# jnetter6/RRTQX_3D

Measured on AMD Instinct MI355X. Metric: collision-checked edges/sec + radius-NN queries/sec at N=200k nodes, 256 obs, higher is better.
Workload: dtype f64; 1 GPU; C4: 3D SimpleEdge N=200k M=256 B=16384; n_nodes=200000, n_obstacles=256, batch_per_gpu=16384, global_batch=16384, obstacle_list=spheres, edge=SimpleEdge, fresh_batch_every_step=True, batch_ring=8

## Files before the change

rrtqx_3d_amd/csrc/kernels_finish.hip:

```cpp
#include "nn_device.hpp"

namespace rrtx {

namespace {

constexpr int kFinThreads = 512;
constexpr int kFinQ = kFinThreads / 32;
constexpr int kBigSort = 2048;
constexpr int kHugeSort = 8192;
constexpr int kFinBins = 2048;
constexpr int kFinCrowd = 128;

struct FinishArgs {
  const int *count;
  int nq, bcap;
  const BktRec *bkt;
  BktRec *tmp;
  const HitRec *ovf;
  long long ovf_cap;
  const Scalars *sc;
  int prescattered;
  int want_nearest_fix;
  int64_t *offsets;
  int64_t *needed;
  int32_t *idx;
  double *dist;
  long long out_cap;
  int32_t *owner;
  int32_t *nearest_idx;
  double *nearest_dist;
  int *qhist;
  int n_qhist;
  unsigned *mailbox;
  const double *q;
  uint8_t *hit_out, *hit_in;
  double r_start;
  NearestIndex ni;
};

template <int KSORT>
struct FinLds {
  long long red[kFinThreads / 64];
  long long off[kFinQ + 1];
  int kfull[kFinQ];
  int todo[kFinQ];
  unsigned todo_mask;
  unsigned empty_mask;
  int gcnt;
  int s_idx[KSORT];
  double s_d2[KSORT];
  unsigned char s_fl[KSORT];
  int bins[kFinBins + 1];
  int mm[2 * (kFinThreads / 64)];
  double r_best[kFinThreads / 64];
  int r_besti[kFinThreads / 64];
  NearestScratch ns;
};

__device__ __forceinline__ BktRec load_rec(const FinishArgs &a, int q, long long b, long long j) {
  if (j < a.bcap) return a.bkt[(size_t)q * (size_t)a.bcap + (size_t)j];
  const unsigned long long *p = reinterpret_cast<const unsigned long long *>(a.tmp + b + j);
  BktRec r;
  const unsigned long long w0 = __hip_atomic_load(p, __ATOMIC_RELAXED, __HIP_MEMORY_SCOPE_AGENT);
  const unsigned long long w1 = __hip_atomic_load(p + 1, __ATOMIC_RELAXED, __HIP_MEMORY_SCOPE_AGENT);
  r.idx = (int)(unsigned)(w0 & 0xffffffffull);
  r.pad = (int)(unsigned)(w0 >> 32);
  r.d2 = __longlong_as_double((long long)w1);
  return r;
}

template <int D, int KSORT>
__global__ __launch_bounds__(kFinThreads, KSORT > kBigSort ? 2 : 8) void nn_finish_kernel(FinishArgs a) {
  __shared__ FinLds<KSORT> sm;
  const int t = threadIdx.x, lane = t & 63;
  const int wave = __builtin_amdgcn_readfirstlane(t >> 6);
  const int hl = t & 31, hw = t >> 5;
  const int q0 = (int)blockIdx.x * kFinQ;
  const int q = q0 + hw;
  const bool qv = q < a.nq;

  for (int k = (int)blockIdx.x * kFinThreads + t; k < a.n_qhist; k += (int)gridDim.x * kFinThreads) a.qhist[k] = 0;
  if (blockIdx.x == 0 && t == 0 && a.mailbox) {
    const unsigned long long tot = a.sc->total;
    a.mailbox[0] = tot > 0xffffffffull ? 0xffffffffu : (unsigned)tot;
  }

  if (hl == 0) sm.todo[hw] = 0;
  if (t == 0) sm.empty_mask = 0u;
  int kfull = 0;
  if (qv) kfull = a.count[q];
  const int kInt = 0x7fffffff;
  BktRec e0, e1;
  e0.idx = kInt; e0.pad = 0; e0.d2 = __builtin_inf();
  e1 = e0;
  if (qv && hl < a.bcap) e0 = a.bkt[(size_t)q * (size_t)a.bcap + (size_t)hl];
  unsigned long long psum = 0;
  if (!a.prescattered) {
    const int4 *c4 = reinterpret_cast<const int4 *>(a.count);
    const int n4 = (int)blockIdx.x * (kFinQ / 4);
#pragma unroll 4
    for (int j = t; j < n4; j += kFinThreads) {
      const int4 v = c4[j];
      psum += (unsigned)v.x + (unsigned)v.y;
      psum += (unsigned)v.z + (unsigned)v.w;
    }
  }
  const bool small = kfull <= 64 && kfull <= a.bcap;
  const int kk = (qv && small) ? kfull : 0;
  if (!(hl < kk)) { e0.idx = kInt; e0.d2 = __builtin_inf(); }
  if (hl + 32 < kk) e1 = a.bkt[(size_t)q * (size_t)a.bcap + (size_t)(hl + 32)];
  __builtin_amdgcn_wave_barrier();

  const int m0 = e0.idx, m1 = e1.idx;
  const double d0 = e0.d2, d1 = e1.d2;
  int r0 = half_rank_below<false>(m0, m0), r1 = 0;
  double nbest = d0;
  int nbest_i = m0;
  if (__ballot(kk > 32) != 0ull) {
    r0 += half_rank_below<true>(m1, m0);
    r1 = half_rank_below<true>(m0, m1) + half_rank_below<false>(m1, m1);
    const bool second = (d1 < d0) | ((d1 == d0) & (m1 < m0));
    nbest = second ? d1 : d0;
    nbest_i = second ? m1 : m0;
  }
  if (a.nearest_idx) {
    const double dm = half_min_no_nan(nbest);
    nbest_i = half_min((nbest == dm) ? nbest_i : kInt);
    nbest = dm;
  }

  if (!a.prescattered) {
    psum = wave_sum_last(psum);
    if (lane == 63) sm.red[wave] = (long long)psum;
  }
  if (qv && hl == 0) {
    sm.kfull[hw] = kfull;
    if (!small) sm.todo[hw] = 1;
  }
  if (!qv && hl == 0) sm.kfull[hw] = 0;
  __syncthreads();
  if (wave == 0) {
    long long p = 0;
    if (a.prescattered) {
      p = a.offsets[q0];
    } else {
      for (int w = 0; w < kFinThreads / 64; ++w) p += sm.red[w];
    }
    const int kf = lane < kFinQ ? sm.kfull[lane] : 0;
    const int td = lane < kFinQ ? sm.todo[lane] : 0;
    static_assert(kFinQ == 16, "the sixteen lengths sit in one DPP row");
    const long long v = (long long)row_incl_scan((unsigned long long)kf);
    if (lane < kFinQ) sm.off[lane] = p + v - kf;
    if (lane == kFinQ - 1) sm.off[kFinQ] = p + v;
    const unsigned long long tmb = __ballot(td != 0);
    if (lane == 0) sm.todo_mask = (unsigned)tmb;
  }
  __syncthreads();
  if (!a.prescattered && t <= kFinQ) {
    const int qq = q0 + t;
    if (qq < a.nq) a.offsets[qq] = sm.off[t];
    if (qq == a.nq) {
      a.offsets[qq] = sm.off[t];
      if (a.needed) *a.needed = sm.off[t];
    }
  }

  {
    const long long b = qv ? sm.off[hw] : 0;
    const bool w0 = hl < kk && b + r0 < a.out_cap, w1 = hl + 32 < kk && b + r1 < a.out_cap;
    const bool near = a.nearest_idx != nullptr;
    if (hl < kk) {
      const double s0 = sqrt_rn(d0);
      if (w0) {
        a.idx[b + r0] = m0;
        a.dist[b + r0] = s0;
        if (a.owner) a.owner[b + r0] = q;
        if (a.hit_out) { a.hit_out[b + r0] = e0.pad & 1; a.hit_in[b + r0] = (e0.pad >> 1) & 1; }
      }
      if (near && m0 == nbest_i && d0 == nbest) { a.nearest_idx[q] = m0; a.nearest_dist[q] = s0; }
    }
    if (hl + 32 < kk) {
      const double s1 = sqrt_rn(d1);
      if (w1) {
        a.idx[b + r1] = m1;
        a.dist[b + r1] = s1;
        if (a.owner) a.owner[b + r1] = q;
        if (a.hit_out) { a.hit_out[b + r1] = e1.pad & 1; a.hit_in[b + r1] = (e1.pad >> 1) & 1; }
      }
      if (near && m1 == nbest_i && d1 == nbest) { a.nearest_idx[q] = m1; a.nearest_dist[q] = s1; }
    }
    if (near && qv && small && hl == 0 && kk == 0) {
      if (a.want_nearest_fix) atomicOr(&sm.empty_mask, 1u << hw);
      else { a.nearest_idx[q] = -1; a.nearest_dist[q] = __builtin_inf(); }
    }
  }
  __syncthreads();

  for (unsigned tm = sm.todo_mask; tm != 0u; tm &= tm - 1u) {
    const int g = __ffs((int)tm) - 1;
    const int qq = q0 + g;
    const long long gb = sm.off[g];
    const int gfull = sm.kfull[g];
    long long ge = gb + gfull;
    if (ge > a.out_cap) ge = a.out_cap;
    const int gk = ge > gb ? (int)(ge - gb) : 0;
    if (!a.prescattered && gfull > a.bcap) {
      if (t == 0) sm.gcnt = 0;
      __syncthreads();
      long long total = (long long)a.sc->total;
      if (total > a.ovf_cap) total = a.ovf_cap;
      for (long long i = t; i < total; i += kFinThreads) {
        const HitRec r = a.ovf[i];
        if ((r.owner & 0x3fffffff) == qq) {
          const long long dst = gb + a.bcap + atomicAdd(&sm.gcnt, 1);
          if (dst < a.out_cap) {
            unsigned long long *p = reinterpret_cast<unsigned long long *>(a.tmp + dst);
            __hip_atomic_store(p, (unsigned long long)(unsigned)r.idx | ((unsigned long long)((unsigned)r.owner >> 30) << 32),
                               __ATOMIC_RELAXED, __HIP_MEMORY_SCOPE_AGENT);
            __hip_atomic_store(p + 1, (unsigned long long)__double_as_longlong(r.d2), __ATOMIC_RELAXED,
                               __HIP_MEMORY_SCOPE_AGENT);
          }
        }
      }
      asm volatile("s_waitcnt vmcnt(0)" ::: "memory");
      __syncthreads();
    }
    double best = __builtin_inf();
    int best_i = 0x7fffffff;
    bool placed = false;
    if (KSORT > kBigSort && gk <= KSORT) {
      constexpr int kEpt = KSORT / kFinThreads;
      int my_idx[kEpt], my_fl[kEpt], my_bin[kEpt], my_in[kEpt];
      double my_d2[kEpt];
      int lo = 0x7fffffff, hi = (int)0x80000000;
#pragma unroll
      for (int e = 0; e < kEpt; ++e) {
        const int i = e * kFinThreads + t;
        my_idx[e] = 0x7fffffff; my_fl[e] = 0; my_d2[e] = __builtin_inf(); my_bin[e] = 0; my_in[e] = 0;
        if (i < gk) {
          const BktRec r = load_rec(a, qq, gb, i);
          my_idx[e] = r.idx; my_d2[e] = r.d2; my_fl[e] = r.pad;
          lo = min(lo, r.idx); hi = max(hi, r.idx);
        }
      }
      for (int k = t; k <= kFinBins; k += kFinThreads) sm.bins[k] = 0;
#pragma unroll
      for (int off = 32; off > 0; off >>= 1) { lo = min(lo, __shfl_xor(lo, off)); hi = max(hi, __shfl_xor(hi, off)); }
      if (lane == 0) { sm.mm[2 * wave] = lo; sm.mm[2 * wave + 1] = hi; }
      __syncthreads();
#pragma unroll
      for (int w = 0; w < kFinThreads / 64; ++w) { lo = min(lo, sm.mm[2 * w]); hi = max(hi, sm.mm[2 * w + 1]); }
      const double scale = (double)kFinBins / ((double)hi - (double)lo + 1.0);
#pragma unroll
      for (int e = 0; e < kEpt; ++e) {
        if (e * kFinThreads + t < gk) {
          int b = (int)(((double)my_idx[e] - (double)lo) * scale);
          b = b < 0 ? 0 : (b > kFinBins - 1 ? kFinBins - 1 : b);
          my_bin[e] = b;
          my_in[e] = atomicAdd(&sm.bins[b], 1);
        }
      }
      __syncthreads();
      {
        static_assert(kFinBins == 4 * kFinThreads, "four bins per thread");
        const int c0 = sm.bins[4 * t], c1 = sm.bins[4 * t + 1], c2 = sm.bins[4 * t + 2], c3 = sm.bins[4 * t + 3];
        int v = c0 + c1 + c2 + c3;
        const int mine = v;
#pragma unroll
        for (int off = 1; off < 64; off <<= 1) {
          const int o = __shfl_up(v, off);
          if (lane >= off) v += o;
        }
        int cmax = max(max(c0, c1), max(c2, c3));
#pragma unroll
        for (int off = 32; off > 0; off >>= 1) cmax = max(cmax, __shfl_xor(cmax, off));
        if (lane == 63) { sm.mm[wave] = v; sm.mm[kFinThreads / 64 + wave] = cmax; }
        __syncthreads();
        int pre = v - mine;
        for (int w = 0; w < wave; ++w) pre += sm.mm[w];
        sm.bins[4 * t] = pre; sm.bins[4 * t + 1] = pre + c0; sm.bins[4 * t + 2] = pre + c0 + c1; sm.bins[4 * t + 3] = pre + c0 + c1 + c2;
        if (t == kFinThreads - 1) sm.bins[kFinBins] = pre + mine;
      }
      int crowd = 0;
#pragma unroll
      for (int w = 0; w < kFinThreads / 64; ++w) crowd = max(crowd, sm.mm[kFinThreads / 64 + w]);
      placed = crowd <= kFinCrowd;
      __syncthreads();
     if (placed) {
      int *t_idx = sm.s_idx;
      int *t_pos = reinterpret_cast<int *>(sm.s_d2);
#pragma unroll
      for (int e = 0; e < kEpt; ++e) {
        if (e * kFinThreads + t < gk) {
          const int p = sm.bins[my_bin[e]] + my_in[e];
          t_idx[p] = my_idx[e];
          t_pos[p] = e * kFinThreads + t;
        }
      }
      __syncthreads();
#pragma unroll
      for (int e = 0; e < kEpt; ++e) {
        const int i = e * kFinThreads + t;
        if (i < gk) {
          const int my = my_idx[e];
          const int s0 = sm.bins[my_bin[e]], s1 = sm.bins[my_bin[e] + 1];
          int rank = s0;
          for (int k = s0; k < s1; ++k) {
            const int v = t_idx[k];
            rank += ((v < my) || (v == my && t_pos[k] < i)) ? 1 : 0;
          }
          const double d2 = my_d2[e];
          a.idx[gb + rank] = my;
          a.dist[gb + rank] = sqrt_rn(d2);
          if (a.owner) a.owner[gb + rank] = qq;
          if ((d2 < best) || (d2 == best && my < best_i)) { best = d2; best_i = my; }
          if (a.hit_out) { a.hit_out[gb + rank] = my_fl[e] & 1; a.hit_in[gb + rank] = (my_fl[e] >> 1) & 1; }
        }
      }
     }
    }
    if (placed) {
    } else if (gk <= KSORT) {
      int n2 = 64;
      while (n2 < gk) n2 <<= 1;
      for (int i = t; i < n2; i += kFinThreads) {
        BktRec r;
        r.idx = 0x7fffffff; r.pad = 0; r.d2 = __builtin_inf();
        if (i < gk) r = load_rec(a, qq, gb, i);
        sm.s_idx[i] = r.idx;
        sm.s_d2[i] = r.d2;
        sm.s_fl[i] = (unsigned char)r.pad;
      }
      __syncthreads();
      for (int size = 2; size <= n2; size <<= 1) {
        for (int stride = size >> 1; stride > 0; stride >>= 1) {
          for (int i = t; i < n2; i += kFinThreads) {
            const int j = i ^ stride;
            if (j > i) {
              const bool up = (i & size) == 0;
              const int aa = sm.s_idx[i], cc = sm.s_idx[j];
              if ((aa > cc) == up) {
                sm.s_idx[i] = cc; sm.s_idx[j] = aa;
                const double da = sm.s_d2[i];
                sm.s_d2[i] = sm.s_d2[j]; sm.s_d2[j] = da;
                const unsigned char fa = sm.s_fl[i];
                sm.s_fl[i] = sm.s_fl[j]; sm.s_fl[j] = fa;
              }
            }
          }
          __syncthreads();
        }
      }
      for (int i0 = 0; i0 < gk; i0 += kFinThreads) {
        const int i = i0 + t;
        const bool act = i < gk;
        int my = 0;
        double d2 = 0.0;
        if (act) {
          my = sm.s_idx[i];
          d2 = sm.s_d2[i];
          a.idx[gb + i] = my;
          a.dist[gb + i] = sqrt_rn(d2);
          if (a.owner) a.owner[gb + i] = qq;
          if ((d2 < best) || (d2 == best && my < best_i)) { best = d2; best_i = my; }
          if (a.hit_out) { const int fl = sm.s_fl[i]; a.hit_out[gb + i] = fl & 1; a.hit_in[gb + i] = (fl >> 1) & 1; }
        }
      }
    } else {
      for (int i0 = 0; i0 < gk; i0 += kFinThreads) {
        const int i = i0 + t;
        const bool act = i < gk;
        int my = 0, rank = 0;
        double d2 = 0.0;
        if (act) {
          const BktRec r = load_rec(a, qq, gb, i);
          my = r.idx; d2 = r.d2;
          for (int j = 0; j < gk; ++j) rank += (load_rec(a, qq, gb, j).idx < my) ? 1 : 0;
          a.idx[gb + rank] = my;
          a.dist[gb + rank] = sqrt_rn(d2);
          if (a.owner) a.owner[gb + rank] = qq;
          if ((d2 < best) || (d2 == best && my < best_i)) { best = d2; best_i = my; }
          if (a.hit_out) { a.hit_out[gb + rank] = r.pad & 1; a.hit_in[gb + rank] = (r.pad >> 1) & 1; }
        }
      }
    }
    if (a.nearest_idx) {
#pragma unroll
      for (int off = 32; off > 0; off >>= 1) {
        const double ob = __shfl_xor(best, off);
        const int oi = __shfl_xor(best_i, off);
        if ((ob < best) || (ob == best && oi < best_i)) { best = ob; best_i = oi; }
      }
      if (lane == 0) { sm.r_best[wave] = best; sm.r_besti[wave] = best_i; }
      __syncthreads();
      if (t == 0) {
        for (int w = 1; w < kFinThreads / 64; ++w)
          if ((sm.r_best[w] < best) || (sm.r_best[w] == best && sm.r_besti[w] < best_i)) {
            best = sm.r_best[w]; best_i = sm.r_besti[w];
          }
        if (gk > 0) { a.nearest_idx[qq] = best_i; a.nearest_dist[qq] = sqrt_rn(best); }
        else if (a.want_nearest_fix) atomicOr(&sm.empty_mask, 1u << g);
        else { a.nearest_idx[qq] = -1; a.nearest_dist[qq] = __builtin_inf(); }
      }
    }
    __syncthreads();
  }

  if (a.nearest_idx && a.want_nearest_fix) {
    for (unsigned em = sm.empty_mask; em != 0u; em &= em - 1u) {
      const int g = __ffs((int)em) - 1;
      const int qq = q0 + g;
      const double ex = a.q[(size_t)qq * D + 0], ey = a.q[(size_t)qq * D + 1], ez = a.q[(size_t)qq * D + 2];
      double ew = 0.0;
      if constexpr (D == 4) ew = a.q[(size_t)qq * D + 3];
      double bs;
      int bi;
      block_nearest<D, kFinThreads>(a.ni, ex, ey, ez, ew, a.r_start, sm.ns, bs, bi);
      if (t == 0) { a.nearest_idx[qq] = bi; a.nearest_dist[qq] = sqrt_rn(bs); }
    }
  }
}

}

int launch_nn_finish(rrtx_ctx *ctx, const FinishLaunch &f) {
  const int D = ctx->dim;
  FinishArgs a;
  a.count = f.count; a.nq = f.nq; a.bcap = f.bcap;
  a.bkt = reinterpret_cast<const BktRec *>(f.bkt);
  a.tmp = reinterpret_cast<BktRec *>(f.tmp);
  a.ovf = reinterpret_cast<const HitRec *>(f.ovf);
  a.ovf_cap = f.ovf_cap;
  a.sc = reinterpret_cast<const Scalars *>(f.scalars);
  a.prescattered = f.prescattered ? 1 : 0;
  a.offsets = f.offsets; a.needed = f.needed;
  a.idx = f.idx; a.dist = f.dist; a.out_cap = f.out_cap;
  a.owner = f.owner; a.nearest_idx = f.nearest_idx; a.nearest_dist = f.nearest_dist;
  a.qhist = f.qhist; a.n_qhist = f.n_qhist;
  a.mailbox = f.mailbox;
  a.q = f.q;
  a.r_start = f.r_start;
  a.want_nearest_fix = (f.nearest_idx && ctx->n_wraps == 0) ? 1 : 0;
  a.ni.sx = ctx->sl_d[0]; a.ni.sy = ctx->sl_d[1]; a.ni.sz = ctx->sl_d[2]; a.ni.sw = ctx->sl_d[D == 4 ? 3 : 2];
  a.ni.sid = ctx->sl_id;
  a.ni.chunk_ext = reinterpret_cast<const ChunkExt *>(ctx->chunk_ext.get());
  a.ni.n_nodes = (int)ctx->n_nodes;
  a.ni.n_chunks = (int)((ctx->n_nodes + kSlabChunk - 1) / kSlabChunk);
  a.hit_out = f.hit_out; a.hit_in = f.hit_in;
  const dim3 grid((unsigned)((f.nq + kFinQ - 1) / kFinQ)), block(kFinThreads);
  const bool huge = f.out_cap / (f.nq > 0 ? f.nq : 1) > 512;
  for_dim(D, [&](auto dc) {
    constexpr int DD = decltype(dc)::value;
    if (huge) hipLaunchKernelGGL((nn_finish_kernel<DD, kHugeSort>), grid, block, 0, ctx->stream, a);
    else hipLaunchKernelGGL((nn_finish_kernel<DD, kBigSort>), grid, block, 0, ctx->stream, a);
  });
  RRTX_HIP(ctx, hipGetLastError());
  return RRTX_OK;
}

}
```

rrtqx_3d_amd/csrc/kernels_nn.hip:

```cpp
#include "collide_device.hpp"
#include "nn_device.hpp"

#include <limits>

namespace rrtx {

namespace {

template <int D>
__global__ __launch_bounds__(kScanThreads) void nn_scan_kernel(
    const double *__restrict__ nx, const double *__restrict__ ny, const double *__restrict__ nz,
    const double *__restrict__ nw, int n_nodes, const typename QRecT<D>::type *__restrict__ copies,
    const int2 *__restrict__ meta, const SlotRec *__restrict__ slots, int n_slots, int tile_q, int n_seg,
    int seg_len, const Scalars *__restrict__ sc, HitSink hs) {
  const int seg = blockIdx.x % n_seg;
  const int tile = blockIdx.x / n_seg;
  const int n_copies = sc->n_copies;
  const int q0 = tile * tile_q;
  if (q0 >= n_copies) return;
  const int q1 = min(q0 + tile_q, n_copies);
  const int lane = threadIdx.x & 63;
  const int wave = threadIdx.x >> 6;
  const int node_begin = seg * seg_len;
  const int node_end = min(n_nodes, node_begin + seg_len);
  const double kNaN = __builtin_nan("");

  for (int base = node_begin + wave * kChunk; base < node_end; base += (kScanThreads / 64) * kChunk) {
    double x[kScanU], y[kScanU], z[kScanU], w[kScanU];
    int id[kScanU];
#pragma unroll
    for (int u = 0; u < kScanU; ++u) {
      id[u] = base + u * 64 + lane;
      bool ok = id[u] < node_end;
      x[u] = ok ? nx[id[u]] : kNaN;
      y[u] = ok ? ny[id[u]] : kNaN;
      z[u] = ok ? nz[id[u]] : kNaN;
      if constexpr (D == 4) w[u] = ok ? nw[id[u]] : kNaN; else w[u] = 0.0;
    }
    for (int q = q0; q < q1; ++q) {
      const typename QRecT<D>::type c = copies[q];
      double s[kScanU];
      bool h[kScanU];
      bool any = false;
#pragma unroll
      for (int u = 0; u < kScanU; ++u) {
        if constexpr (D == 4) s[u] = sq4(c.x, c.y, c.z, c.w, x[u], y[u], z[u], w[u]);
        else s[u] = sq3(c.x, c.y, c.z, x[u], y[u], z[u]);
        h[u] = s[u] < c.thr;
        any = any || h[u];
      }
      if (__builtin_expect(__ballot(any) != 0ull, 0)) {
        const int2 m = meta[q];
#pragma unroll
        for (int u = 0; u < kScanU; ++u) {
          bool hu = h[u];
          if (m.y > 0 && hu)
            hu = !seen_by_earlier_slot<D>(slots, n_slots, m.x, m.y, id[u], x[u], y[u], z[u], w[u]);
          emit_hit(hs, hu, m.x, id[u], s[u]);
        }
      }
    }
  }
  (void)lane;
}

constexpr int kMaxQBuckets = 4096;
template <int D>
__global__ __launch_bounds__(256) void nn_place_kernel(
    const typename QRecT<D>::type *__restrict__ copies, const int2 *__restrict__ meta, const int2 *__restrict__ cb,
    const int *__restrict__ qhist, int n_buckets, const Scalars *__restrict__ sc,
    const unsigned long long *__restrict__ node_absmax, double ox, double oy, double oz, double ow,
    typename QRecT<D>::type *__restrict__ copies_s, int2 *__restrict__ meta_s,
    typename QRecFT<D>::type *__restrict__ copies_f) {
  __shared__ int start[kMaxQBuckets];
  __shared__ int wsum[4];
  {
    const int t = threadIdx.x, lane = t & 63, wave = t >> 6;
    static_assert(kMaxQBuckets == 256 * 16, "sixteen counters per thread");
    const int per = (n_buckets + 255) / 256;
    const int b0 = min(t * per, n_buckets), b1 = min(b0 + per, n_buckets);
    int h[16];
    if (per == 16) {
      const int4 *h4 = reinterpret_cast<const int4 *>(qhist + b0);
#pragma unroll
      for (int k = 0; k < 4; ++k) { const int4 v4 = h4[k]; h[4 * k] = v4.x; h[4 * k + 1] = v4.y; h[4 * k + 2] = v4.z; h[4 * k + 3] = v4.w; }
    } else {
#pragma unroll
      for (int k = 0; k < 16; ++k) h[k] = (b0 + k < b1) ? qhist[b0 + k] : 0;
    }
    int local = 0;
#pragma unroll
    for (int k = 0; k < 16; ++k) local += h[k];
    int v = local;
#pragma unroll
    for (int off = 1; off < 64; off <<= 1) {
      const int o = __shfl_up(v, off);
      if (lane >= off) v += o;
    }
    if (lane == 63) wsum[wave] = v;
    __syncthreads();
    int prefix = v - local;
    for (int w = 0; w < wave; ++w) prefix += wsum[w];
#pragma unroll
    for (int k = 0; k < 16; ++k)
      if (b0 + k < b1) { start[b0 + k] = prefix; prefix += h[k]; }
    __syncthreads();
  }
  int i = blockIdx.x * blockDim.x + threadIdx.x;
  const int n_copies = sc->n_copies;
  if (i >= n_copies) {
    if (i < ((n_copies + kQPI - 1) / kQPI) * kQPI) copies_f[i] = never_pass_qrecf<D>();
    return;
  }
  const int2 b = cb[i];
  const int dst = start[b.x] + b.y;
  if ((unsigned)dst >= (unsigned)n_copies) return;
  const typename QRecT<D>::type c = copies[i];
  unsigned long long am = max(*node_absmax, sc->q_absmax);
  copies_s[dst] = c;
  meta_s[dst] = meta[i];
  copies_f[dst] = make_qrecf<D>(c, __longlong_as_double((long long)am), ox, oy, oz, ow);
}

constexpr int kEvSlack = 2048;

template <int D, bool LM, class Emit>
__device__ __forceinline__ void confirm_entry(bool has, int2 en, int n_nodes, const ConfirmArgs &a, const Emit &emit,
                                              const typename QRecT<D>::type *tile_copies = nullptr, int tile_q0 = 0) {
  const typename QRecT<D>::type *__restrict__ copies = static_cast<const typename QRecT<D>::type *>(a.copies);
  typename QRecT<D>::type ce;
  ce.x = 0.0; ce.y = 0.0; ce.z = 0.0; ce.thr = 0.0;
  if constexpr (D == 4) ce.w = 0.0;
  int2 m = make_int2(0, 0);
  const int p0 = has ? en.y : 0;
  if (has) {
    ce = tile_copies ? tile_copies[en.x - tile_q0] : copies[en.x];
    if (Emit::kNeedsOwner || a.n_slots > 1) m = a.meta[en.x];
  }
  constexpr int kH = kScanFU / 2;
#pragma unroll 1
  for (int hv = 0; hv < 2; ++hv) {
    double ex[kH], ey[kH], ez[kH], ew[kH];
    int nid[kH];
    if constexpr (LM) {
      if (a.pos_id) {
        const int4 vi = *reinterpret_cast<const int4 *>(a.pos_id + p0 + kH * hv);
        nid[0] = vi.x; nid[1] = vi.y; nid[2] = vi.z; nid[3] = vi.w;
      } else {
#pragma unroll
        for (int u = 0; u < kH; ++u) nid[u] = p0 + kH * hv + u;
      }
      const double2 *rx = reinterpret_cast<const double2 *>(a.nx + p0 + kH * hv);
      const double2 *ry = reinterpret_cast<const double2 *>(a.ny + p0 + kH * hv);
      const double2 *rz = reinterpret_cast<const double2 *>(a.nz + p0 + kH * hv);
      const double2 *rw = reinterpret_cast<const double2 *>(a.nw + p0 + kH * hv);
#pragma unroll
      for (int v = 0; v < kH / 2; ++v) {
        const double2 vx = rx[v], vy = ry[v], vz = rz[v];
        ex[2 * v] = vx.x; ex[2 * v + 1] = vx.y;
        ey[2 * v] = vy.x; ey[2 * v + 1] = vy.y;
        ez[2 * v] = vz.x; ez[2 * v + 1] = vz.y;
        if constexpr (D == 4) { const double2 vw = rw[v]; ew[2 * v] = vw.x; ew[2 * v + 1] = vw.y; }
        else { ew[2 * v] = 0.0; ew[2 * v + 1] = 0.0; }
      }
    } else {
#pragma unroll
      for (int u = 0; u < kH; ++u) {
        const int pos = p0 + 64 * (kH * hv + u);
        const int pc = (pos < n_nodes) ? pos : 0;
        ex[u] = a.nx[pc]; ey[u] = a.ny[pc]; ez[u] = a.nz[pc];
        if constexpr (D == 4) ew[u] = a.nw[pc]; else ew[u] = 0.0;
        nid[u] = pos;
      }
    }
    double s[kH];
    unsigned hm = 0u;
#pragma unroll
    for (int u = 0; u < kH; ++u) {
      const int pos = LM ? p0 + kH * hv + u : p0 + 64 * (kH * hv + u);
      if constexpr (D == 4) s[u] = sq4(ce.x, ce.y, ce.z, ce.w, ex[u], ey[u], ez[u], ew[u]);
      else s[u] = sq3(ce.x, ce.y, ce.z, ex[u], ey[u], ez[u]);
      bool hu = has && pos < n_nodes && (s[u] < ce.thr);
      if (m.y > 0 && hu)
        hu = !seen_by_earlier_slot<D>(a.slots, a.n_slots, m.x, m.y, nid[u], ex[u], ey[u], ez[u], ew[u]);
      hm |= (hu ? 1u : 0u) << u;
    }
    if constexpr (Emit::kBatch) {
      static_assert(kH == 4, "batch emitters take four nodes at a time");
      emit.batch(en.x, m.x, hm, nid, s);
    } else {
      while (__ballot(hm != 0u) != 0ull) {
        const bool h = hm != 0u;
        const int uu = h ? (__ffs((int)hm) - 1) : 0;
        hm &= hm - 1u;
        double hs2 = s[0];
        int hid = nid[0];
#pragma unroll
        for (int u = 1; u < kH; ++u) { hs2 = (uu == u) ? s[u] : hs2; hid = (uu == u) ? nid[u] : hid; }
        emit(h, en.x, m.x, hid, hs2);
      }
    }
  }
}

constexpr int kConfirmParts = 4;
template <int D, bool LM>
__global__ __launch_bounds__(256) void nn_confirm_kernel(ConfirmArgs a, const int2 *__restrict__ ev,
                                                         const int *__restrict__ ev_cnt, int n_slices,
                                                         int slice_cap, int n_nodes) {
  const int lane = threadIdx.x & 63;
  const int gw = __builtin_amdgcn_readfirstlane((int)blockIdx.x * (int)(blockDim.x >> 6) + (int)(threadIdx.x >> 6));
  const int w = gw / kConfirmParts, part = gw % kConfirmParts;
  if (w >= n_slices) return;
  const int cnt = ev_cnt[w];
  const int2 *__restrict__ mine = ev + (size_t)w * (size_t)slice_cap;
  for (int e0 = 64 * part; e0 < cnt; e0 += 64 * kConfirmParts) {
    const int e = e0 + lane;
    const bool has = e < cnt;
    int2 en = make_int2(0, 0);
    if (has) en = mine[e];
    confirm_entry<D, LM>(has, en, n_nodes, a, GlobalEmit{a.hs});
  }
}


template <int D>
__device__ __forceinline__ typename QRecFT<D>::type uniform_qrecf(const typename QRecFT<D>::type &f) {
  typename QRecFT<D>::type u = f;
  u.x = __int_as_float(__builtin_amdgcn_readfirstlane(__float_as_int(f.x)));
  u.y = __int_as_float(__builtin_amdgcn_readfirstlane(__float_as_int(f.y)));
  u.z = __int_as_float(__builtin_amdgcn_readfirstlane(__float_as_int(f.z)));
  if constexpr (D == 4) u.w = __int_as_float(__builtin_amdgcn_readfirstlane(__float_as_int(f.w)));
  u.thr = __int_as_float(__builtin_amdgcn_readfirstlane(__float_as_int(f.thr)));
  return u;
}
template <int D, int MODE, bool LQ = false>
__device__ __forceinline__ void scan_chunk_f32(const float *__restrict__ fx, const float *__restrict__ fy,
                                               const float *__restrict__ fz, const float *__restrict__ fw,
                                               const float *__restrict__ fpp, const int base, const int node_end,
                                               const typename QRecFT<D>::type *__restrict__ copies_f, const int q0,
                                               const int q1, int2 *__restrict__ mine, int &wn,
                                               const unsigned p_lane = 0u, const unsigned long long vm = ~0ull,
                                               const typename QRecFT<D>::type *lq = nullptr) {
  const int lane = threadIdx.x & 63;
  const float kInf = __builtin_inff();
  constexpr bool LM = MODE != 0;
  float x[kScanFU], y[kScanFU], z[kScanFU], w[kScanFU], pp[kScanFU];
  const unsigned p0 = (MODE == 2) ? p_lane : (unsigned)(base + 8 * lane);
  if constexpr (LM) {
    const float4 *rx = reinterpret_cast<const float4 *>(fx + p0);
    const float4 *ry = reinterpret_cast<const float4 *>(fy + p0);
    const float4 *rz = reinterpret_cast<const float4 *>(fz + p0);
    const float4 *rw = reinterpret_cast<const float4 *>(fw + p0);
    const float4 *rp = reinterpret_cast<const float4 *>(fpp + p0);
#pragma unroll
    for (int v = 0; v < 2; ++v) {
      const float4 vx = rx[v], vy = ry[v], vz = rz[v], vp = rp[v];
      x[4 * v] = vx.x; x[4 * v + 1] = vx.y; x[4 * v + 2] = vx.z; x[4 * v + 3] = vx.w;
      y[4 * v] = vy.x; y[4 * v + 1] = vy.y; y[4 * v + 2] = vy.z; y[4 * v + 3] = vy.w;
      z[4 * v] = vz.x; z[4 * v + 1] = vz.y; z[4 * v + 2] = vz.z; z[4 * v + 3] = vz.w;
      pp[4 * v] = vp.x; pp[4 * v + 1] = vp.y; pp[4 * v + 2] = vp.z; pp[4 * v + 3] = vp.w;
      if constexpr (D == 4) {
        const float4 vw = rw[v];
        w[4 * v] = vw.x; w[4 * v + 1] = vw.y; w[4 * v + 2] = vw.z; w[4 * v + 3] = vw.w;
      } else {
        w[4 * v] = 0.f; w[4 * v + 1] = 0.f; w[4 * v + 2] = 0.f; w[4 * v + 3] = 0.f;
      }
    }
#pragma unroll
    for (int u = 0; u < kScanFU; ++u)
      if ((int)p0 + u >= node_end) { x[u] = 0.f; y[u] = 0.f; z[u] = 0.f; w[u] = 0.f; pp[u] = kInf; }
  } else {
#pragma unroll
    for (int u = 0; u < kScanFU; ++u) {
      const int id = base + u * 64 + lane;
      const bool ok = id < node_end;
      const unsigned idc = (unsigned)(ok ? id : node_end - 1);
      x[u] = fx[idc];
      y[u] = fy[idc];
      z[u] = fz[idc];
      if constexpr (D == 4) w[u] = fw[idc]; else w[u] = 0.f;
      pp[u] = ok ? fpp[idc] : kInf;
    }
  }
  for (int q = q0; q < q1; q += kQPI) {
    typename QRecFT<D>::type c[kQPI];
#pragma unroll
    for (int k = 0; k < kQPI; ++k) {
      if constexpr (LQ) c[k] = uniform_qrecf<D>(lq[q - q0 + k]);
      else c[k] = copies_f[q + k];
    }
    unsigned long long mk[kQPI];
    unsigned long long anym = 0ull;
#pragma unroll
    for (int k = 0; k < kQPI; ++k) {
      float t[kScanFU];
      screen8<D>(c[k], x, y, z, w, pp, t);
      const float m1 = fminf(fminf(t[0], t[1]), t[2]);
      const float m2 = fminf(fminf(t[3], t[4]), t[5]);
      const float m3 = fminf(fminf(t[6], t[7]), m1);
      const float tmin = fminf(m2, m3);
      mk[k] = __ballot(!(tmin > c[k].thr));
      if constexpr (MODE == 2) mk[k] &= vm;
      anym |= mk[k];
    }
    if (anym != 0ull) {
#pragma unroll
      for (int k = 0; k < kQPI; ++k) {
        if (mk[k] == 0ull || q + k >= q1) continue;
        const unsigned before = __builtin_amdgcn_mbcnt_hi((unsigned)(mk[k] >> 32),
                                                          __builtin_amdgcn_mbcnt_lo((unsigned)mk[k], 0u));
        if ((mk[k] >> lane) & 1ull)
          mine[wn + (int)before] = make_int2(q + k, LM ? (int)p0 : base + lane);
        wn += __popcll(mk[k]);
      }
    }
  }
}

template <int D, bool LM, class Emit>
__device__ __forceinline__ void drain_slice_to(const int2 *__restrict__ mine, int &wn, int n_nodes, const ConfirmArgs &a,
                                               const Emit &emit, const typename QRecT<D>::type *tile_copies, int tile_q0) {
  const int lane = threadIdx.x & 63;
  __builtin_amdgcn_fence(__ATOMIC_SEQ_CST, "workgroup");
  for (int e0 = 0; e0 < wn; e0 += 64) {
    const int e = e0 + lane;
    const bool has = e < wn;
    int2 en = make_int2(0, 0);
    if (has) en = mine[e];
    confirm_entry<D, LM>(has, en, n_nodes, a, emit, tile_copies, tile_q0);
  }
  wn = 0;
}

template <int D, bool LM>
__device__ __forceinline__ void drain_slice(const int2 *__restrict__ mine, int &wn, int n_nodes,
                                            const ConfirmArgs *__restrict__ ca) {
  const int lane = threadIdx.x & 63;
  __builtin_amdgcn_fence(__ATOMIC_SEQ_CST, "workgroup");
  const ConfirmArgs a = *ca;
  for (int e0 = 0; e0 < wn; e0 += 64) {
    const int e = e0 + lane;
    const bool has = e < wn;
    int2 en = make_int2(0, 0);
    if (has) en = mine[e];
    confirm_entry<D, LM>(has, en, n_nodes, a, GlobalEmit{a.hs});
  }
  wn = 0;
}

template <int D>
__global__ __launch_bounds__(kScanThreads, 5) void nn_scan_f32_kernel(
    const float *__restrict__ fx, const float *__restrict__ fy, const float *__restrict__ fz,
    const float *__restrict__ fw, const float *__restrict__ fpp, int n_nodes,
    const typename QRecFT<D>::type *__restrict__ copies_f, int tile_q, int n_seg, int seg_len,
    const Scalars *__restrict__ sc, int2 *__restrict__ ev, int *__restrict__ ev_cnt, int slice_cap,
    const ConfirmArgs *__restrict__ ca) {
  const int n_copies = sc->n_copies;
  const int lane = threadIdx.x & 63;
  const int wave = threadIdx.x >> 6;
  const int slice = __builtin_amdgcn_readfirstlane((int)blockIdx.x * (kScanThreads / 64) + wave);
  int2 *__restrict__ mine = ev + (size_t)slice * (size_t)slice_cap;
  int wn = 0;
  const int n_tiles = (n_copies + tile_q - 1) / tile_q;
  const int n_items = n_tiles * n_seg;
  for (int item = blockIdx.x; item < n_items; item += gridDim.x) {
    const int seg = item % n_seg;
    const int tile = item / n_seg;
    const int q0 = tile * tile_q;
    const int q1 = min(q0 + tile_q, n_copies);
    const int node_begin = seg * seg_len;
    const int node_end = min(n_nodes, node_begin + seg_len);
    for (int base = node_begin + wave * kChunkF; base < node_end; base += (kScanThreads / 64) * kChunkF) {
      if (wn + 64 * tile_q > slice_cap) drain_slice<D, false>(mine, wn, n_nodes, ca);
      scan_chunk_f32<D, 0>(fx, fy, fz, fw, fpp, base, node_end, copies_f, q0, q1, mine, wn);
    }
  }
  if (lane == 0) ev_cnt[slice] = wn;
}

constexpr int kTileB = 16;
constexpr int kTbLcap = 96;
constexpr int kTbList = 1024;
constexpr int kTbSlack = 512;

constexpr int kTbGroups = 1024;
template <int D>
struct TileLds {
  int list[kTbList];
  int n_list;
  int glist[kTbGroups];
  int n_groups, gmode;
  double zlo, zhi;
  int wcnt[kScanThreads / 64];
  double lo, hi, ylo, yhi;
  int lcnt[kTileB];
  typename QRecT<D>::type cp[kTileB];
  typename QRecFT<D>::type cf[kTileB];
  int own[kTileB];
  BktRec hrec[kTileB][kTbLcap];
  int snl[kTileB];
  int sok[kTileB];
  int ssl[kTileB][kSphListCap];
  SphRec ssr[kTileB][kSphListCap];
};

struct TileGrid {
  const SlabParams *sp;
  const int *cell_start;
  int n_sorted_chunks;
  int kz;
  int groups;
};

template <int D>
__device__ __forceinline__ bool tile_edge_needed(const ExtendDev &x, const TileLds<D> &sm, int cl, double d2) {
  const double len = sqrt_rn(d2);
  const bool quick = sm.snl[cl] == 0 && sm.sok[cl] != 0 && len > 0.0 && len <= x.r_bound && len < 1e29;
  return !quick && x.m > 0;
}
template <int D>
__device__ __forceinline__ int tile_edge_eval(const ExtendDev &x, const TileLds<D> &sm, bool need, int cl,
                                              const double4 nd, double d2) {
  if (__ballot(need) == 0ull) return 0;
  const typename QRecT<D>::type c = sm.cp[cl];
  bool ho, hi;
  edge_flags(x, need, c.x, c.y, c.z, nd.x, nd.y, nd.z, sqrt_rn(d2), sm.snl[cl], sm.ssl[cl], ho, hi, sm.ssr[cl]);
  return (ho ? 1 : 0) | (hi ? 2 : 0);
}
template <int D>
__device__ __forceinline__ int tile_edge_flags(const ExtendDev &x, const TileLds<D> &sm, bool h, int cl, int id,
                                               double d2) {
  const bool need = h && tile_edge_needed<D>(x, sm, cl, d2);
  if (__ballot(need) == 0ull) return 0;
  double4 nd = make_double4(0.0, 0.0, 0.0, 0.0);
  if (need) nd = x.naos[id];
  return tile_edge_eval<D>(x, sm, need, cl, nd, d2);
}

template <int D, bool EXT>
struct TileEmit {
  static constexpr bool kNeedsOwner = false;
  static constexpr bool kBatch = true;
  __device__ __forceinline__ void batch(int q, int , unsigned hm, const int *id, const double *d2) const {
    const int cl = hm ? q - q0 : 0;
    int base = 0;
    if (hm) base = atomicAdd(&sm.lcnt[cl], __popc(hm));
    unsigned spill = 0u;
#pragma unroll
    for (int u = 0; u < 4; ++u) {
      const bool b = (hm >> u) & 1u;
      if (__ballot(b) == 0ull) continue;
      const int slot = base + __popc(hm & ((1u << u) - 1u));
      if (b && slot < kTbLcap) {
        BktRec br;
        br.idx = id[u]; br.pad = 0; br.d2 = d2[u];
        sm.hrec[cl][slot] = br;
      }
      spill |= (b && slot >= kTbLcap) ? (1u << u) : 0u;
    }
    if (__ballot(spill != 0u) != 0ull) {
#pragma unroll 1
      for (int u = 0; u < 4; ++u) {
        const bool sp = (spill >> u) & 1u;
        if (__ballot(sp) == 0ull) continue;
        int owner = 0, flags = 0;
        if (sp) owner = meta ? meta[q].x : sm.own[cl];
        if constexpr (EXT) flags = tile_edge_flags<D>(x, sm, sp, cl, id[u], d2[u]);
        emit_hits_grouped(hs, sp, owner, id[u], d2[u], flags);
      }
    }
  }
  TileLds<D> &sm;
  const HitSink &hs;
  const int2 *meta;
  const ExtendDev &x;
  int q0;
  __device__ __forceinline__ void operator()(bool h, int q, int , int id, double d2) const {
    const int cl = h ? q - q0 : 0;
    int slot = 0;
    if (h) slot = atomicAdd(&sm.lcnt[cl], 1);
    const bool in_lds = h && slot < kTbLcap;
    if (in_lds) {
      BktRec br;
      br.idx = id; br.pad = 0; br.d2 = d2;
      sm.hrec[cl][slot] = br;
    }
    const bool spill = h && !in_lds;
    if (__ballot(spill) != 0ull) {
      int owner = 0, flags = 0;
      if (spill) owner = meta ? meta[q].x : sm.own[cl];
      if constexpr (EXT) flags = tile_edge_flags<D>(x, sm, spill, cl, id, d2);
      emit_hits_grouped(hs, spill, owner, id, d2, flags);
    }
  }
};

__device__ __forceinline__ int lane_here() {
  int l = (int)(threadIdx.x & 63);
  asm volatile("" : "+v"(l));
  return l;
}
__device__ __forceinline__ int wshfl_i(int v, int src_lane) { return __builtin_amdgcn_ds_bpermute(src_lane << 2, v); }
template <bool MAX>
__device__ __forceinline__ int wave_scan_incl(int v, const int identity) {
#define RRTX_SCAN_STEP(ctrl, rows)                                                              \
  {                                                                                             \
    const int o = __builtin_amdgcn_update_dpp(identity, v, ctrl, rows, 0xf, false);             \
    v = MAX ? max(v, o) : v + o;                                                                \
  }
  RRTX_SCAN_STEP(0x111, 0xf) RRTX_SCAN_STEP(0x112, 0xf) RRTX_SCAN_STEP(0x114, 0xf) RRTX_SCAN_STEP(0x118, 0xf)
  RRTX_SCAN_STEP(0x142, 0xa) RRTX_SCAN_STEP(0x143, 0xc)
#undef RRTX_SCAN_STEP
  return v;
}
template <int N>
__device__ __forceinline__ double row_up_d(double v) {
  const long long b = __double_as_longlong(v);
  const int lo = __builtin_amdgcn_update_dpp((int)(b & 0xffffffffll), (int)(b & 0xffffffffll), 0x100 + N, 0xf, 0xf, false);
  const int hi = __builtin_amdgcn_update_dpp((int)(b >> 32), (int)(b >> 32), 0x100 + N, 0xf, 0xf, false);
  return __longlong_as_double(((long long)hi << 32) | (long long)(unsigned)lo);
}
__device__ __forceinline__ int wave_prev(int v, const int first) {
  return __builtin_amdgcn_update_dpp(first, v, 0x138, 0xf, 0xf, false);
}
__device__ __forceinline__ double wshfl_d(double v, int src_lane) {
  const long long b = __double_as_longlong(v);
  const int lo = __builtin_amdgcn_ds_bpermute(src_lane << 2, (int)(b & 0xffffffffll));
  const int hi = __builtin_amdgcn_ds_bpermute(src_lane << 2, (int)(b >> 32));
  return __longlong_as_double(((long long)hi << 32) | (long long)(unsigned)lo);
}

#ifdef RRTX_TILE_CLOCKS
__device__ unsigned long long g_tile_clk[4096 * 16];
#define RRTX_TILE_CLK_AT(thread, k) do { if (t == (thread)) g_tile_clk[(blockIdx.x & 4095) * 16 + (k)] = wall_clock64(); } while (0)
#else
#define RRTX_TILE_CLK_AT(thread, k) do { } while (0)
#endif
#define RRTX_TILE_CLK(k) RRTX_TILE_CLK_AT(0, k)

struct TilePlace {
  const int *qhist;
  const void *tab;
  const int2 *spill_key;
  int n_buckets, capb, spill_base, n_tab;
};

__device__ __forceinline__ void load_qhist16(const int *__restrict__ qhist, int per, int b0, int b1, int *h) {
  static_assert(kMaxQBuckets == 256 * 16, "sixteen counters per thread");
  if (per == 16) {
    const int4 *h4 = reinterpret_cast<const int4 *>(qhist + b0);
#pragma unroll
    for (int k = 0; k < 4; ++k) { const int4 v4 = h4[k]; h[4 * k] = v4.x; h[4 * k + 1] = v4.y; h[4 * k + 2] = v4.z; h[4 * k + 3] = v4.w; }
  } else {
#pragma unroll
    for (int k = 0; k < 16; ++k) h[k] = (b0 + k < b1) ? qhist[b0 + k] : 0;
  }
}

template <int D, bool EXT, bool SL, bool ONE>
__global__ __launch_bounds__(kScanThreads, 4) void nn_tile_kernel(
    const float *__restrict__ fx, const float *__restrict__ fy, const float *__restrict__ fz,
    const float *__restrict__ fw, const float *__restrict__ fpp, int n_nodes, int n_chunks,
    const ChunkExt *__restrict__ chunk_ext, const typename QRecT<D>::type *__restrict__ copies_s, const typename QRecFT<D>::type *__restrict__ copies_f,
    const Scalars *__restrict__ sc, int n_parts, int2 *__restrict__ ev, int slice_cap,
    const ConfirmArgs a, const ConfirmArgs *__restrict__ ca, const TileGrid tg, const ExtendDev x,
    int *__restrict__ visits, const int n_copies_known, const TilePlace tp) {
  __shared__ TileLds<D> sm;
  const int t = threadIdx.x, lane = t & 63;
  const int wave = __builtin_amdgcn_readfirstlane(t >> 6);
  const int part = blockIdx.x % n_parts;
  const int n_copies = n_copies_known >= 0 ? n_copies_known : sc->n_copies;
  const int n_tiles = (n_copies + kTileB - 1) / kTileB;
  const int slice = (int)blockIdx.x * (kScanThreads / 64) + wave;
  int2 *__restrict__ mine = ev + (size_t)slice * (size_t)slice_cap;
  const int2 *__restrict__ blk = ev + (size_t)blockIdx.x * (kScanThreads / 64) * (size_t)slice_cap;
  int visited = 0;

  const int n_slots = (int)gridDim.x / n_parts;
  const int slot = (int)blockIdx.x / n_parts;
  const int my = (n_slots % 8 == 0) ? (slot % 8) * (n_slots / 8) + slot / 8 : slot;
  for (int tile = my; tile < n_tiles; tile += n_slots) {
    const int q0 = tile * kTileB;
    const int q1 = min(q0 + kTileB, n_copies);
    int wn = 0;

    RRTX_TILE_CLK(0);
    int slot = -1;
    if constexpr (SL) {
      int tq = t;
      asm volatile("" : "+v"(tq));
      const int per = (tp.n_buckets + 255) / 256;
      {
        const int b0 = min(tq * per, tp.n_buckets), b1 = min(b0 + per, tp.n_buckets);
        int h[16];
        load_qhist16(tp.qhist, per, b0, b1, h);
        int local = 0;
#pragma unroll
        for (int k = 0; k < 16; ++k) local += h[k];
        const int incl = wave_scan_incl<false>(local, 0);
        if (lane == 63) sm.wcnt[wave] = incl;
        sm.list[kTileB + tq] = incl - local;
      }
      __syncthreads();
      RRTX_TILE_CLK(11);
      if (wave == 0) {
        const int pos = q0 + lane;
        int rk = -1, bk = 0;
        if (pos < q1) {
          const int w1 = sm.wcnt[0], w2 = w1 + sm.wcnt[1], w3 = w2 + sm.wcnt[2];
          auto start_of = [&](int T) {
            const int w = T >> 6;
            return sm.list[kTileB + T] + (w == 0 ? 0 : (w == 1 ? w1 : (w == 2 ? w2 : w3)));
          };
          int T = 0;
#pragma unroll
          for (int st = 128; st > 0; st >>= 1)
            if (start_of(T + st) <= pos) T += st;
          int p = start_of(T);
          const int b0 = min(T * per, tp.n_buckets), b1 = min(b0 + per, tp.n_buckets);
          int h[16];
          load_qhist16(tp.qhist, per, b0, b1, h);
#pragma unroll
          for (int k = 0; k < 16; ++k) {
            const bool in = pos >= p && pos < p + h[k];
            bk = in ? b0 + k : bk;
            rk = in ? pos - p : rk;
            p += h[k];
          }
          if (rk >= 0 && rk < tp.capb) slot = bk * tp.capb + rk;
        }
        const unsigned long long need = __ballot(rk >= tp.capb);
        if (need != 0ull) {
          const int n_sp = min(sc->n_spill, n_copies);
          unsigned long long todo = need;
          for (int j0 = 0; j0 < n_sp && todo != 0ull; j0 += 64) {
            const int j = j0 + lane;
            const int2 key = j < n_sp ? tp.spill_key[j] : make_int2(-1, -1);
            unsigned long long rem = todo;
            while (rem != 0ull) {
              const int l = __ffsll((long long)rem) - 1;
              rem &= rem - 1ull;
              const int kb = __builtin_amdgcn_readlane(bk, l), kr = __builtin_amdgcn_readlane(rk, l);
              const unsigned long long m = __ballot(key.x == kb && key.y == kr);
              if (m != 0ull) {
                if (lane == l) slot = tp.spill_base + j0 + __ffsll((long long)m) - 1;
                todo &= ~(1ull << l);
              }
            }
          }
        }
      }
    }

    if (t < kTileB) sm.lcnt[t] = 0;
    if (wave == 0) {
      double lo = __builtin_inf(), hi = -__builtin_inf(), ylo = __builtin_inf(), yhi = -__builtin_inf();
      double zlo = __builtin_inf(), zhi = -__builtin_inf();
      if constexpr (SL) {
        if (lane >= q1 - q0 && lane < kTileB) sm.cf[lane] = never_pass_qrecf<D>();
      }
      if (q0 + lane < q1) {
        typename QRecT<D>::type c;
        if constexpr (SL) {
          if ((unsigned)slot < (unsigned)tp.n_tab) {
            const QSlotRec<D> rec = static_cast<const QSlotRec<D> *>(tp.tab)[slot];
            c = rec.q;
            sm.cf[lane] = rec.f;
            sm.own[lane] = rec.owner;
          } else {
            c.x = 0.0; c.y = 0.0; c.z = 0.0; c.thr = -1.0;
            if constexpr (D == 4) { c.w = 0.0; c.pad0 = 0.0; c.pad1 = 0.0; c.pad2 = 0.0; }
            sm.cf[lane] = never_pass_qrecf<D>();
            sm.own[lane] = -1;
          }
        } else {
          c = copies_s[q0 + lane];
        }
        sm.cp[lane] = c;
        if constexpr (EXT) {
          const double rb = x.r_bound >= 0.0 ? x.r_bound : 0.0;
          const double pmax = fmax(fmax(fabs(c.x), fabs(c.y)), fabs(c.z));
          const double base_b = rb + 1e-12 * (pmax + 1.0);
          const bool usable = (pmax < 1e29) && (c.x == c.x) && (c.y == c.y) && (c.z == c.z) && (base_b < 1e29);
          sm.sok[lane] = (usable && x.r_bound >= 0.0) ? 1 : 0;
        }
        const bool can_hit = (c.thr > 0.0) && (c.x - c.x == 0.0) && (c.y - c.y == 0.0) && (c.z - c.z == 0.0);
        if (can_hit) {
          const double R = sqrt_rn(c.thr) * (1.0 + 1e-15);
          const double xa = c.x - R, xb = c.x + R, ya = c.y - R, yb = c.y + R, za = c.z - R, zb = c.z + R;
          lo = xa - (fabs(xa) * 4.5e-16 + 1e-300);
          hi = xb + (fabs(xb) * 4.5e-16 + 1e-300);
          ylo = ya - (fabs(ya) * 4.5e-16 + 1e-300);
          yhi = yb + (fabs(yb) * 4.5e-16 + 1e-300);
          zlo = za - (fabs(za) * 4.5e-16 + 1e-300);
          zhi = zb + (fabs(zb) * 4.5e-16 + 1e-300);
        }
      }
      {
        static_assert(kTileB == 16, "reach reduction covers lanes 0..15");
#define RRTX_REACH_STEP(N)                                                                   \
        lo = fmin(lo, row_up_d<N>(lo)); hi = fmax(hi, row_up_d<N>(hi));                     \
        ylo = fmin(ylo, row_up_d<N>(ylo)); yhi = fmax(yhi, row_up_d<N>(yhi));               \
        zlo = fmin(zlo, row_up_d<N>(zlo)); zhi = fmax(zhi, row_up_d<N>(zhi));
        RRTX_REACH_STEP(8) RRTX_REACH_STEP(4) RRTX_REACH_STEP(2) RRTX_REACH_STEP(1)
#undef RRTX_REACH_STEP
      }
      if (lane == 0) {
        sm.lo = lo; sm.hi = hi; sm.ylo = ylo; sm.yhi = yhi; sm.zlo = zlo; sm.zhi = zhi;
        sm.n_list = 0; sm.n_groups = 0; sm.gmode = 0;
      }
    }
    __syncthreads();
    RRTX_TILE_CLK(1);
    const double lo = sm.lo, hi = sm.hi, ylo = sm.ylo, yhi = sm.yhi;
    bool gmode_w0 = false;
    if (lo <= hi) {
      for (int cb = 0; ONE || cb < n_chunks; cb += kTbList) {
        const int ce = ONE ? n_chunks : min(cb + kTbList, n_chunks);
        if (wave == 0) {
          const int w_end = min(ce, tg.n_sorted_chunks);
          if (cb == 0 && tg.groups && w_end > 0) {
            const SlabParams sp = *tg.sp;
            const int Kz = tg.kz;
            const int cx0 = slab_of(lo, sp.x0, sp.inv_wx, sp.Kx), cx1 = slab_of(hi, sp.x0, sp.inv_wx, sp.Kx);
            const int cy0 = slab_of(ylo, sp.y0, sp.inv_wy, sp.Ky), cy1 = slab_of(yhi, sp.y0, sp.inv_wy, sp.Ky);
            const int cz0 = slab_of(sm.zlo, sp.z0, sp.inv_wz, Kz), cz1 = slab_of(sm.zhi, sp.z0, sp.inv_wz, Kz);
            const int wdt = cx1 - cx0 + 1, nc = (lo <= hi) ? wdt * (cy1 - cy0 + 1) : 0;
            const int g_end = tg.n_sorted_chunks * (kChunkF / 8);
            int listed_to = -1, G = 0;
            for (int i0 = 0; i0 < nc && G <= kTbGroups; i0 += 64) {
              const int i = i0 + lane;
              int g0 = 0, g1 = -1;
              if (i < nc) {
                const int row = i / wdt, col = i - row * wdt;
                const int cy = cy0 + row;
                const int c = cy * sp.Kx + ((cy & 1) ? (sp.Kx - 1 - cx1) : cx0) + col;
                const int p0 = tg.cell_start[c * Kz + cz0], p1 = tg.cell_start[c * Kz + cz1 + 1];
                if (p1 > p0) { g0 = p0 >> 3; g1 = min((p1 - 1) >> 3, g_end - 1); }
              }
              const int run = wave_scan_incl<true>(g1, -1);
              const int before = max(wave_prev(run, listed_to), listed_to);
              g0 = max(g0, before + 1);
              const int cnt = max(g1 - g0 + 1, 0);
              const int inc = wave_scan_incl<false>(cnt, 0);
              const int at = G + inc - cnt;
              for (int j = 0; j < cnt; ++j)
                if (at + j < kTbGroups) sm.glist[at + j] = g0 + j;
              G += __builtin_amdgcn_readlane(inc, 63);
              listed_to = max(listed_to, __builtin_amdgcn_readlane(run, 63));
            }
            gmode_w0 = G <= kTbGroups;
            if (lane == 0) { sm.n_groups = gmode_w0 ? G : 0; sm.gmode = gmode_w0 ? 1 : 0; }
          }
          if (cb < w_end && !gmode_w0 && lo <= hi) {
            const SlabParams sp = *tg.sp;
            const int Kz = tg.kz;
            const int cx0 = slab_of(lo, sp.x0, sp.inv_wx, sp.Kx), cx1 = slab_of(hi, sp.x0, sp.inv_wx, sp.Kx);
            const int cy0 = slab_of(ylo, sp.y0, sp.inv_wy, sp.Ky), cy1 = slab_of(yhi, sp.y0, sp.inv_wy, sp.Ky);
            int listed_to = cb - 1;
            for (int r0 = cy0; r0 <= cy1; r0 += 64) {
              const int cy = r0 + lane;
              int ca_ = 0, cb_ = -1;
              if (cy <= cy1) {
                const int base = cy * sp.Kx;
                const int c_first = base + ((cy & 1) ? (sp.Kx - 1 - cx1) : cx0);
                const int c_last = base + ((cy & 1) ? (sp.Kx - 1 - cx0) : cx1);
                const int p0 = tg.cell_start[c_first * Kz], p1 = tg.cell_start[(c_last + 1) * Kz];
                if (p1 > p0) { ca_ = max(p0 / kChunkF, cb); cb_ = min((p1 - 1) / kChunkF, w_end - 1); }
              }
              int run = cb_;
              const int l = lane_here();
#pragma unroll
              for (int off = 1; off < 64; off <<= 1) {
                const int o = wshfl_i(run, l >= off ? l - off : l);
                if (lane >= off) run = max(run, o);
              }
              int before = wshfl_i(run, l >= 1 ? l - 1 : l);
              if (lane == 0) before = listed_to;
              before = max(before, listed_to);
              ca_ = max(ca_, before + 1);
              const int cnt = cb_ - ca_ + 1;
              if (cnt > 0) {
                const int at = atomicAdd(&sm.n_list, cnt);
                for (int j = 0; j < cnt; ++j) sm.list[at + j] = ca_ + j;
              }
              listed_to = max(listed_to, __builtin_amdgcn_readlane(run, 63));
            }
          }
        } else if (EXT && wave >= 2) {
          if (cb == 0) {
            static_assert(kTileB * kSphListCap == 128, "two waves: one lane per (copy, list slot)");
            int ts = t - 128;
            asm volatile("" : "+v"(ts));
            const int cl = ts / kSphListCap, ls = ts % kSphListCap;
            int n = 0, j = 0;
            if (cl < q1 - q0) {
              const int owner = SL ? sm.own[cl] : a.meta[q0 + cl].x;
              if (owner >= 0) {
                const SampleList *rec = x.lists + owner;
                n = rec->n; j = rec->list[ls];
              }
            }
            if (ls == 0) sm.snl[cl] = n;
            if (ls < n) { sm.ssl[cl][ls] = j; sm.ssr[cl][ls] = x.sph[j]; }
          }
        } else {
          const int nt = EXT ? 64 : 192;
          for (int c = max(cb, tg.n_sorted_chunks) + (t - 64); c < ce; c += nt) {
            const ChunkExt cx = chunk_ext[c];
            if (dec_ord(cx.xhi) >= lo && dec_ord(cx.xlo) <= hi && dec_ord(cx.yhi) >= ylo && dec_ord(cx.ylo) <= yhi)
              sm.list[atomicAdd(&sm.n_list, 1)] = c;
          }
        }
        RRTX_TILE_CLK_AT(0, 8);
        RRTX_TILE_CLK_AT(64, 9);
        RRTX_TILE_CLK_AT(128, 10);
        __syncthreads();
        RRTX_TILE_CLK(2);
        const int nl = sm.n_list;
        if (cb == 0 && sm.gmode) {
          const int G = sm.n_groups, n_gu = (G + 63) >> 6;
          for (int k = wave;; k += kScanThreads / 64) {
            const int u = part + n_parts * k;
            if (u >= n_gu) break;
            const int gi = 64 * u + lane;
            const bool valid = gi < G;
            const unsigned p_lane = valid ? 8u * (unsigned)sm.glist[gi] : 0u;
            if (wn + 64 * kTileB > slice_cap) {
              const TileEmit<D, EXT> emit_now{sm, a.hs, SL ? nullptr : a.meta, x, q0};
              drain_slice_to<D, true>(mine, wn, n_nodes, a, emit_now, sm.cp, q0);
            }
            scan_chunk_f32<D, 2, SL>(fx, fy, fz, fw, fpp, 0, n_nodes, copies_f, q0, q1, mine, wn, p_lane, __ballot(valid),
                                     sm.cf);
            visited += min(64, G - 64 * u);
          }
        }
        for (int i = wave; i < nl; i += kScanThreads / 64) {
          const int chunk = __builtin_amdgcn_readfirstlane(sm.list[i]);
          if (n_parts > 1 && chunk % n_parts != part) continue;
          {
            const ChunkExt cx = chunk_ext[chunk];
            if (!(dec_ord(cx.xhi) >= lo && dec_ord(cx.xlo) <= hi && dec_ord(cx.yhi) >= ylo && dec_ord(cx.ylo) <= yhi))
              continue;
          }
          if (wn + 64 * kTileB > slice_cap) {
            const TileEmit<D, EXT> emit_now{sm, a.hs, SL ? nullptr : a.meta, x, q0};
            drain_slice_to<D, true>(mine, wn, n_nodes, a, emit_now, sm.cp, q0);
          }
          scan_chunk_f32<D, 1, SL>(fx, fy, fz, fw, fpp, chunk * kChunkF, n_nodes, copies_f, q0, q1, mine, wn, 0u, ~0ull,
                                   sm.cf);
          visited += kChunkF / 8;
        }
        if constexpr (ONE) break;
        if (ce < n_chunks) {
          __syncthreads();
          if (t == 0) sm.n_list = 0;
          __syncthreads();
        }
      }
    }
    RRTX_TILE_CLK(3);
    if (lane == 0) sm.wcnt[wave] = wn;
    __builtin_amdgcn_fence(__ATOMIC_SEQ_CST, "workgroup");
    __syncthreads();
    RRTX_TILE_CLK(4);
    const TileEmit<D, EXT> emit{sm, a.hs, SL ? nullptr : a.meta, x, q0};
    const int c0 = sm.wcnt[0], c1 = c0 + sm.wcnt[1], c2 = c1 + sm.wcnt[2], total = c2 + sm.wcnt[3];
    for (int e0 = 0; e0 < total; e0 += kScanThreads) {
      const int e = e0 + t;
      const bool has = e < total;
      int2 en = make_int2(0, 0);
      if (has) {
        const int w = (e >= c0) + (e >= c1) + (e >= c2);
        const int local = e - (w == 0 ? 0 : (w == 1 ? c0 : (w == 2 ? c1 : c2)));
        en = blk[(size_t)w * (size_t)slice_cap + local];
      }
      if (__ballot(has) != 0ull) confirm_entry<D, true>(has, en, n_nodes, a, emit, sm.cp, q0);
    }
    __syncthreads();
    RRTX_TILE_CLK(5);
    {
      constexpr int kPerWave = kTileB / (kScanThreads / 64);
      const int nc = q1 - q0;
      int my_n = 0, my_owner = 0, my_base = 0;
      if (lane < kPerWave) {
        const int cl = (lane >> 1) * (kTileB / 2) + wave * 2 + (lane & 1);
        if (cl < nc) {
          my_n = min(sm.lcnt[cl], kTbLcap);
          if (my_n > 0) {
            my_owner = SL ? sm.own[cl] : a.meta[q0 + cl].x;
            my_base = atomicAdd(&a.hs.count[my_owner], my_n);
          }
        }
      }
      const int half = lane >> 5, hl = lane & 31;
      for (int i = 0; i < kPerWave / 2; ++i) {
        const int s = i * 2 + half;
        const int cl = i * (kTileB / 2) + wave * 2 + half;
        const int n = __shfl(my_n, s), owner = __shfl(my_owner, s), base = __shfl(my_base, s);
        const int nmax = max(n, wshfl_i(n, lane_here() ^ 32));
        for (int j0 = 0; j0 < nmax; j0 += 32) {
          const int j = j0 + hl;
          const bool h = j < n;
          BktRec br;
          br.idx = 0; br.pad = 0; br.d2 = 0.0;
          if (h) br = sm.hrec[cl][j];
          int flags = 0;
          if constexpr (EXT) flags = tile_edge_flags<D>(x, sm, h, h ? cl : 0, br.idx, br.d2);
          place_hit(a.hs, h, owner, base + j, br.idx, br.d2, flags);
        }
      }
    }
    RRTX_TILE_CLK(6);
    if constexpr (!ONE) __syncthreads();
    RRTX_TILE_CLK(7);
    if constexpr (ONE) break;
  }
  if (lane == 0) visits[slice] = visited;
}

__global__ __launch_bounds__(256) void nn_blocksum_kernel(const int *__restrict__ count, int nq,
                                                          long long *__restrict__ block_sum) {
  __shared__ long long wsum[4];
  const int i = blockIdx.x * blockDim.x + threadIdx.x;
  long long v = (i < nq) ? (long long)count[i] : 0ll;
#pragma unroll
  for (int off = 32; off > 0; off >>= 1) v += __shfl_xor(v, off);
  if ((threadIdx.x & 63) == 0) wsum[threadIdx.x >> 6] = v;
  __syncthreads();
  if (threadIdx.x == 0) block_sum[blockIdx.x] = wsum[0] + wsum[1] + wsum[2] + wsum[3];
}

__global__ __launch_bounds__(256) void nn_offsets_kernel(const int *__restrict__ count, int nq,
                                                         const long long *__restrict__ block_sum,
                                                         int64_t *__restrict__ offsets,
                                                         int *__restrict__ cursor,
                                                         int64_t *__restrict__ needed, int *__restrict__ qhist,
                                                         int n_qhist) {
  __shared__ long long red[4];
  __shared__ long long wave_tot[4];
  const int t = threadIdx.x, lane = t & 63, wave = t >> 6;
  for (int k = blockIdx.x * 256 + t; k < n_qhist; k += gridDim.x * 256) qhist[k] = 0;
  long long p = 0;
  if (block_sum) {
    for (int j = t; j < (int)blockIdx.x; j += 256) p += block_sum[j];
  } else {
    const int4 *c4 = reinterpret_cast<const int4 *>(count);
    const int n4 = (int)blockIdx.x * 64;
#pragma unroll 4
    for (int j = t; j < n4; j += 256) {
      const int4 v = c4[j];
      p += (long long)v.x + v.y + v.z + v.w;
    }
  }
#pragma unroll
  for (int off = 32; off > 0; off >>= 1) p += __shfl_xor(p, off);
  if (lane == 0) red[wave] = p;
  const int i = blockIdx.x * 256 + t;
  const long long c = (i < nq) ? (long long)count[i] : 0ll;
  long long v = c;
#pragma unroll
  for (int off = 1; off < 64; off <<= 1) {
    long long o = __shfl_up(v, off);
    if (lane >= off) v += o;
  }
  if (lane == 63) wave_tot[wave] = v;
  __syncthreads();
  long long prefix = red[0] + red[1] + red[2] + red[3];
  for (int w = 0; w < wave; ++w) prefix += wave_tot[w];
  if (i < nq) {
    offsets[i] = prefix + v - c;
    cursor[i] = 0;
  }
  if (i == nq - 1) {
    offsets[nq] = prefix + v;
    if (needed) *needed = (int64_t)(prefix + v);
  }
}

__global__ void nn_scatter_kernel(const HitRec *__restrict__ recs, long long cap,
                                  const Scalars *__restrict__ sc, const int64_t *__restrict__ offsets,
                                  int *__restrict__ cursor, int bcap, BktRec *__restrict__ tmp, long long out_cap) {
  long long total = (long long)sc->total;
  if (total > cap) total = cap;
  for (long long i = (long long)blockIdx.x * blockDim.x + threadIdx.x; i < total;
       i += (long long)gridDim.x * blockDim.x) {
    HitRec r = recs[i];
    const int owner = r.owner & 0x3fffffff;
    long long dst = offsets[owner] + bcap + atomicAdd(&cursor[owner], 1);
    if (dst < out_cap) {
      BktRec br;
      br.idx = r.idx; br.pad = (int)((unsigned)r.owner >> 30); br.d2 = r.d2;
      tmp[dst] = br;
    }
  }
}

}

namespace {

static_assert(kMaxQBuckets == 64 * 64 && kMaxQBuckets == 16 * 16 * 16, "g2 stops at 64, g3 at 16: n_buckets fits");
static_assert(kTbSlack >= 0 && kEvSlack >= 0, "a drained slice holds the worst case of the next screen step");
static_assert(kTileQFilter % kQPI == 0 && kTileQExact % kQPI == 0 && 128 % kQPI == 0, "kQPI copy records per read");

struct RadiusPlan {
  bool use_filter;
  bool use_cull;
  bool slot_route;
  bool fuse;
  bool prescatter;
  int nq, n_nodes, n_chunks;
  int n_slots;
  size_t n_copies_max;
  long long rec_cap;
  int tile_q, n_tiles;
  int n_seg, seg_len;
  int g2, g3;
  int n_buckets;
  int capb;
  int spill_base;
  int n_tab;
  int bcap;
  int n_parts;
  unsigned scan_grid;
  int n_slices;
  bool straight;
  int slice_cap;
};

RadiusPlan plan_radius(const rrtx_ctx *ctx, int nq, int64_t cap, unsigned prev_overflow, bool want_extend) {
  RadiusPlan p{};
  const TuneBits tune = tune_bits(ctx);
  p.nq = nq; p.n_nodes = (int)ctx->n_nodes; p.n_slots = 1 << ctx->n_wraps;
  p.n_copies_max = (size_t)nq * p.n_slots;
  p.rec_cap = (long long)(cap > 0 ? cap : 1);
  p.n_chunks = (p.n_nodes + kSlabChunk - 1) / kSlabChunk;
  p.use_filter = ctx->opt_nn_filter != 0;
  p.use_cull = p.use_filter && (ctx->opt_nn_cull == 2 || (ctx->opt_nn_cull == 1 && p.n_nodes >= 8192));
  p.slot_route = p.use_cull && p.n_slots == 1 && !tune.place_pass;
  p.fuse = want_extend && p.use_cull && ctx->dim == 3 && p.n_slots == 1;
  p.prescatter = nq > 65536 || prev_overflow > 8192u;

  p.tile_q = p.use_filter ? kTileQFilter : kTileQExact;
  if (ctx->opt_tile_q > 0) p.tile_q = (ctx->opt_tile_q + kQPI - 1) / kQPI * kQPI;
  if (p.use_filter && p.tile_q > 128) p.tile_q = 128;
  p.n_tiles = (int)((p.n_copies_max + p.tile_q - 1) / p.tile_q);

  p.g2 = 1; p.g3 = 1; p.n_buckets = 1; p.n_parts = 1;
  if (p.use_cull) {
    while (p.g2 * p.g2 < (long long)(p.n_copies_max / 16) && p.g2 * p.g2 < kMaxQBuckets) p.g2 *= 2;
    p.g3 = (int)std::lround(std::cbrt((double)p.n_copies_max / 4.0));
    if (p.g3 < 1) p.g3 = 1;
    if (tune.g3_side) p.g3 = tune.g3_side;
    if (p.g3 > 16) p.g3 = 16;
    if (tune.xy_order) p.g3 = 1;
    p.n_buckets = std::max(p.g2 * p.g2, p.g3 * p.g3 * p.g3);
  }
  if (p.slot_route) {
    const long long min_b = std::max(1ll, std::min((long long)p.g2 * p.g2, (long long)p.g3 * p.g3 * p.g3));
    const long long avg = ((long long)p.n_copies_max + min_b - 1) / min_b;
    p.capb = (int)std::min(128ll, std::max(8ll, (2 * avg + 8 + 3) / 4 * 4));
    p.spill_base = p.n_buckets * p.capb;
    p.n_tab = p.spill_base + (int)p.n_copies_max;
  }

  long long bcap = (p.rec_cap + nq - 1) / nq * ctx->bkt_mult;
  while (bcap > 16 && bcap * nq > (1ll << 30)) bcap /= 2;
  bcap = (bcap + 7) / 8 * 8;
  p.bcap = (int)std::min(std::max(bcap, 8ll), 1ll << 24);

  const int chunk = p.use_filter ? kChunkF : kChunk;
  const int wg_nodes = (kScanThreads / 64) * chunk;
  const int max_seg = (p.n_nodes + wg_nodes - 1) / wg_nodes;
  const int want_seg = ((p.use_filter ? ctx->opt_scan_items : 4096) + p.n_tiles - 1) / p.n_tiles;
  p.n_seg = std::max(1, std::min(want_seg, max_seg));
  if (p.n_seg >= 8) p.n_seg = p.n_seg / 8 * 8;
  p.seg_len = round_up((p.n_nodes + p.n_seg - 1) / p.n_seg, chunk);
  p.n_seg = (p.n_nodes + p.seg_len - 1) / p.seg_len;
  p.scan_grid = (unsigned)p.n_tiles * (unsigned)p.n_seg;
  if (p.use_cull) {
    const int n_tiles_b = (int)((p.n_copies_max + kTileB - 1) / kTileB);
    p.n_parts = std::min(64, (1024 + n_tiles_b - 1) / n_tiles_b);
    p.scan_grid = (unsigned)std::min(4096ll, (long long)n_tiles_b * p.n_parts);
    p.slice_cap = 64 * kTileB + kTbSlack;
    p.straight = (long long)n_tiles_b * p.n_parts <= 4096 && p.n_chunks <= kTbList && !tune.loop_form;
  } else if (p.use_filter) {
    const unsigned pg = std::max(8u, (unsigned)ctx->opt_scan_blocks / 8u * 8u);
    p.scan_grid = std::min(p.scan_grid, pg);
    p.slice_cap = 64 * p.tile_q + kEvSlack;
  }
  if (p.use_filter) p.n_slices = (int)p.scan_grid * (kScanThreads / 64);
  return p;
}

int radius_workspaces(rrtx_ctx *ctx, const RadiusPlan &p) {
  hipStream_t st = ctx->stream;
  const size_t nc = p.n_copies_max;
  const size_t qrec_bytes = (ctx->dim == 4) ? sizeof(QRec4) : sizeof(QRec3);
  RRTX_HIP(ctx, ctx->ws_slots.ensure(nc * sizeof(SlotRec)));
  RRTX_HIP(ctx, ctx->ws_counts.ensure(((size_t)p.nq * 3 + 2) * sizeof(int)));
  if (!ctx->ws_scalars.p) {
    RRTX_HIP(ctx, ctx->ws_scalars.ensure(2 * sizeof(Scalars)));
    RRTX_HIP(ctx, hipMemsetAsync(ctx->ws_scalars.p, 0, 2 * sizeof(Scalars), st));
  }
  RRTX_HIP(ctx, ctx->ws_recs.ensure((size_t)p.rec_cap * sizeof(HitRec)));
  RRTX_HIP(ctx, ctx->ws_tmp.ensure((size_t)p.rec_cap * sizeof(BktRec)));
  if (!ctx->mailbox.p) {
    RRTX_HIP(ctx, ctx->mailbox.alloc(64, hipHostMallocMapped));
    std::memset(ctx->mailbox.p, 0, 64);
  }
  if (!p.slot_route) {
    const size_t qf_bytes = (ctx->dim == 4) ? sizeof(QRecF4) : sizeof(QRecF3);
    RRTX_HIP(ctx, ctx->ws_copies.ensure(nc * qrec_bytes));
    RRTX_HIP(ctx, ctx->ws_copy_meta.ensure(nc * sizeof(int2)));
    if (p.use_filter) RRTX_HIP(ctx, ctx->ws_copies_f.ensure((nc + kQPI) * qf_bytes));
    if (p.use_cull) RRTX_HIP(ctx, ctx->ws_copies_s.ensure(nc * qrec_bytes));
    if (p.use_cull) RRTX_HIP(ctx, ctx->ws_meta_s.ensure(nc * sizeof(int2)));
  }
  if (p.use_cull) {
    int rc = slab_refresh(ctx, (long long)((nc + 15) / 16));
    if (rc) return rc;
    if (!ctx->ws_qhist.p) {
      RRTX_HIP(ctx, ctx->ws_qhist.ensure(sizeof(int) * (size_t)(kMaxQBuckets + 1)));
      RRTX_HIP(ctx, hipMemsetAsync(ctx->ws_qhist.p, 0, sizeof(int) * (size_t)(kMaxQBuckets + 1), st));
    }
    RRTX_HIP(ctx, ctx->ws_cb.ensure(sizeof(int2) * nc));
    const size_t rec_bytes = (ctx->dim == 4) ? sizeof(QSlotRec<4>) : sizeof(QSlotRec<3>);
    if (p.slot_route) RRTX_HIP(ctx, ctx->ws_qslot.ensure((size_t)p.n_tab * rec_bytes));
  }
  RRTX_HIP(ctx, ctx->ws_bkt.ensure((size_t)p.nq * (size_t)p.bcap * sizeof(BktRec)));
  if (p.fuse) RRTX_HIP(ctx, ctx->ws_sph_lists.ensure((size_t)p.nq * sizeof(SampleList)));
  RRTX_HIP(ctx, ctx->ws_confirm_args.ensure(sizeof(ConfirmArgs)));
  if (p.use_filter) {
    RRTX_HIP(ctx, ctx->ws_ev_a.ensure((size_t)p.n_slices * (size_t)p.slice_cap * sizeof(int2)));
    RRTX_HIP(ctx, ctx->ws_ev_cnt.ensure((size_t)p.n_slices * sizeof(int)));
  }
  if (p.prescatter) RRTX_HIP(ctx, ctx->ws_bsum.ensure(sizeof(long long) * (size_t)((p.nq + 255) / 256)));
  return RRTX_OK;
}

struct RadiusArgs {
  Scalars *sc;
  int *count, *cursor;
  int *qhist; int2 *cbk;
  ConfirmArgs ca, *ca_dev;
  PackFused pf; QSlots qs; ExtendDev xd;
  PackSamples ps;
};

void radius_args(rrtx_ctx *ctx, const RadiusPlan &p, int flip, const ExtendFuse *ext, RadiusArgs &d) {
  const int wi = ctx->dim == 4 ? 3 : 2;
  std::memset(&d, 0, sizeof(d));
  d.sc = ctx->ws_scalars.as<Scalars>() + flip;
  d.count = ctx->ws_counts.as<int>();
  d.cursor = d.count + p.nq + 1;
  if (p.use_cull) { d.qhist = ctx->ws_qhist.as<int>(); d.cbk = ctx->ws_cb.as<int2>(); }
  if (p.slot_route) {
    d.qs.capb = p.capb; d.qs.spill_base = p.spill_base;
    d.qs.tab = ctx->ws_qslot.p; d.qs.spill_key = d.cbk; d.qs.node_absmax = ctx->d_absmax.as<unsigned long long>();
  }
  HitSink &hs = d.ca.hs;
  hs.count = d.count; hs.bkt = ctx->ws_bkt.as<BktRec>(); hs.bcap = p.bcap;
  hs.recs = ctx->ws_recs.as<HitRec>(); hs.cap = p.rec_cap; hs.sc = d.sc;
  const DevArray<double> *pd = p.use_cull ? ctx->sl_d : ctx->nodes;
  d.ca.nx = pd[0]; d.ca.ny = pd[1]; d.ca.nz = pd[2]; d.ca.nw = pd[wi];
  d.ca.copies = p.slot_route ? nullptr : (p.use_cull ? ctx->ws_copies_s.p : ctx->ws_copies.p);
  d.ca.meta = p.slot_route ? nullptr : (p.use_cull ? ctx->ws_meta_s.as<int2>() : ctx->ws_copy_meta.as<int2>());
  d.ca.slots = ctx->ws_slots.as<SlotRec>(); d.ca.pos_id = p.use_cull ? ctx->sl_id : nullptr; d.ca.n_slots = p.n_slots;
  d.ca_dev = ctx->ws_confirm_args.as<ConfirmArgs>();
  d.pf.count = d.count; d.pf.sc_next = ctx->ws_scalars.as<Scalars>() + (flip ^ 1); d.pf.ca_dst = d.ca_dev;
  d.pf.nx = ctx->nodes[0]; d.pf.ny = ctx->nodes[1]; d.pf.nz = ctx->nodes[2]; d.pf.nw = ctx->nodes[wi];
  d.pf.sph = nullptr; d.pf.m_sph = -1; d.pf.root_rule = ctx->opt_root_rule;
  d.xd.r_bound = -1.0;
  if (p.fuse) {
    const SphView &S = ctx->sph_view;
    d.xd.sph = S.rec; d.xd.stab = reinterpret_cast<const SampleSph *>(S.sample);
    d.xd.reach_f = S.reach_f; d.xd.naos = reinterpret_cast<const double4 *>(ctx->nodes_aos.get());
    d.xd.ox = ctx->origin[0]; d.xd.oy = ctx->origin[1]; d.xd.oz = ctx->origin[2]; d.xd.m = S.m;
    d.xd.r_bound = (ext->r >= 0.0 && d.xd.m > 0) ? ext->r * (1.0 + 1e-12) : -1.0;
    d.xd.sample_unsafe = ext->sample_unsafe;
    d.pf.sph = d.xd.sph; d.pf.m_sph = d.xd.m;
    d.xd.lists = ctx->ws_sph_lists.as<SampleList>();
    d.ps.x = d.xd; d.ps.out = ctx->ws_sph_lists.as<SampleList>();
  }
}

void radius_place_or_prep(rrtx_ctx *ctx, const RadiusPlan &p, const RadiusArgs &d) {
  const dim3 grid((unsigned)((p.n_copies_max + kQPI + 255) / 256)), block(256);
  const unsigned long long *absmax = ctx->d_absmax.as<unsigned long long>();
  for_dim(ctx->dim, [&](auto dc) {
    constexpr int D = decltype(dc)::value;
    using Q = typename QRecT<D>::type;
    using QF = typename QRecFT<D>::type;
    if (p.use_cull)
      hipLaunchKernelGGL(nn_place_kernel<D>, grid, block, 0, ctx->stream, ctx->ws_copies.as<Q>(),
                         ctx->ws_copy_meta.as<int2>(), d.cbk, d.qhist, p.n_buckets, d.sc, absmax, ctx->origin[0],
                         ctx->origin[1], ctx->origin[2], ctx->origin[3], ctx->ws_copies_s.as<Q>(),
                         ctx->ws_meta_s.as<int2>(), ctx->ws_copies_f.as<QF>());
    else
      hipLaunchKernelGGL(nn_filter_prep_kernel<D>, grid, block, 0, ctx->stream, ctx->ws_copies.as<Q>(), d.sc, absmax,
                         (int)p.n_copies_max, ctx->origin[0], ctx->origin[1], ctx->origin[2], ctx->origin[3],
                         ctx->ws_copies_f.as<QF>());
  });
}

void radius_scan_tiles(rrtx_ctx *ctx, const RadiusPlan &p, const RadiusArgs &d) {
  TileGrid tg;
  tg.sp = ctx->ws_slab_params.as<SlabParams>();
  tg.cell_start = ctx->ws_slab_start.as<int>();
  tg.n_sorted_chunks = (ctx->ws_slab_params.p && ctx->ws_slab_start.p) ? (int)(ctx->sl_n_sorted / kSlabChunk) : 0;
  tg.kz = ctx->sl_kz > 0 ? ctx->sl_kz : 1;
  tg.groups = (tg.kz > 1 && !tune_bits(ctx).whole_chunks) ? 1 : 0;
  TilePlace tpl;
  tpl.qhist = d.qhist; tpl.tab = d.qs.tab; tpl.spill_key = d.qs.spill_key;
  tpl.n_buckets = p.n_buckets; tpl.capb = p.capb; tpl.spill_base = p.spill_base; tpl.n_tab = p.n_tab;
  const int wi = ctx->dim == 4 ? 3 : 2;
#define RRTX_TILE_LAUNCH_F(DD, EE, SS, OO)                                                                             \
  hipLaunchKernelGGL((nn_tile_kernel<DD, EE, SS, OO>), dim3(p.scan_grid), dim3(kScanThreads), 0, ctx->stream,          \
                     ctx->sl_f[0], ctx->sl_f[1], ctx->sl_f[2], ctx->sl_f[wi], ctx->sl_pp, p.n_nodes, p.n_chunks,       \
                     reinterpret_cast<const ChunkExt *>(ctx->chunk_ext.get()),                                               \
                     SS ? nullptr : ctx->ws_copies_s.as<typename QRecT<DD>::type>(),                                   \
                     SS ? nullptr : ctx->ws_copies_f.as<typename QRecFT<DD>::type>(), d.sc, p.n_parts,                 \
                     ctx->ws_ev_a.as<int2>(), p.slice_cap, d.ca, d.ca_dev, tg, d.xd, ctx->ws_ev_cnt.as<int>(),         \
                     p.n_slots == 1 ? p.nq : -1, tpl)
#define RRTX_TILE_LAUNCH(DD, EE, SS)                                                                                   \
  do { if (p.straight) RRTX_TILE_LAUNCH_F(DD, EE, SS, true); else RRTX_TILE_LAUNCH_F(DD, EE, SS, false); } while (0)
  for_dim(ctx->dim, [&](auto dc) {
    constexpr int D = decltype(dc)::value;
    if constexpr (D == 3) {
      if (p.fuse) {
        if (p.slot_route) RRTX_TILE_LAUNCH(3, true, true);
        else RRTX_TILE_LAUNCH(3, true, false);
        return;
      }
    }
    if (p.slot_route) RRTX_TILE_LAUNCH(D, false, true);
    else RRTX_TILE_LAUNCH(D, false, false);
  });
#undef RRTX_TILE_LAUNCH
#undef RRTX_TILE_LAUNCH_F
}

void radius_scan_brute(rrtx_ctx *ctx, const RadiusPlan &p, const RadiusArgs &d) {
  int2 *ev = ctx->ws_ev_a.as<int2>();
  int *ev_cnt = ctx->ws_ev_cnt.as<int>();
  const dim3 grid(p.scan_grid), block(kScanThreads), cgrid((unsigned)(((long long)p.n_slices * kConfirmParts + 3) / 4));
  for_dim(ctx->dim, [&](auto dc) {
    constexpr int D = decltype(dc)::value;
    constexpr int wi = D == 4 ? 3 : 2;
    if (p.use_filter) {
      hipLaunchKernelGGL(nn_scan_f32_kernel<D>, grid, block, 0, ctx->stream, ctx->nodes_f[0], ctx->nodes_f[1],
                         ctx->nodes_f[2], ctx->nodes_f[wi], ctx->nodes_pp, p.n_nodes,
                         ctx->ws_copies_f.as<typename QRecFT<D>::type>(), p.tile_q, p.n_seg, p.seg_len, d.sc, ev, ev_cnt,
                         p.slice_cap, d.ca_dev);
      hipLaunchKernelGGL((nn_confirm_kernel<D, false>), cgrid, dim3(256), 0, ctx->stream, d.ca, ev, ev_cnt, p.n_slices,
                         p.slice_cap, p.n_nodes);
    } else {
      hipLaunchKernelGGL(nn_scan_kernel<D>, grid, block, 0, ctx->stream, ctx->nodes[0], ctx->nodes[1], ctx->nodes[2],
                         ctx->nodes[wi], p.n_nodes, ctx->ws_copies.as<typename QRecT<D>::type>(),
                         ctx->ws_copy_meta.as<int2>(), ctx->ws_slots.as<SlotRec>(), p.n_slots, p.tile_q, p.n_seg,
                         p.seg_len, d.sc, d.ca.hs);
    }
  });
}

void radius_prescatter(rrtx_ctx *ctx, const RadiusPlan &p, const RadiusArgs &d, int64_t *offsets_dev,
                       int64_t *needed_dev, int64_t cap) {
  hipStream_t st = ctx->stream;
  long long *bsum = ctx->ws_bsum.as<long long>();
  const int nblk = (p.nq + 255) / 256;
  const long long *bsum_arg = nullptr;
  if (p.nq > 65536) {
    hipLaunchKernelGGL(nn_blocksum_kernel, dim3(nblk), dim3(256), 0, st, d.count, p.nq, bsum);
    bsum_arg = bsum;
  }
  hipLaunchKernelGGL(nn_offsets_kernel, dim3(nblk), dim3(256), 0, st, d.count, p.nq, bsum_arg, offsets_dev, d.cursor,
                     needed_dev, (int *)nullptr, 0);
  hipLaunchKernelGGL(nn_scatter_kernel, dim3(1024), dim3(256), 0, st, ctx->ws_recs.as<HitRec>(), p.rec_cap, d.sc,
                     offsets_dev, d.cursor, p.bcap, ctx->ws_tmp.as<BktRec>(), (long long)cap);
}

}

int launch_nn_radius(rrtx_ctx *ctx, const double *q_dev, const double *r_dev_thr_lt, double r_scalar, int nq,
                     int64_t *offsets_dev, int32_t *idx_dev, double *dist_dev, int64_t cap,
                     int64_t *needed_dev, int32_t *owner_dev, int32_t *nearest_idx_dev,
                     double *nearest_dist_dev, ExtendFuse *ext) {
  if (ext) ext->fused = false;
  if (ctx->n_nodes <= 0) return fail(ctx, RRTX_E_STATE, "radius search on an empty tree");
  if (nq <= 0) return RRTX_OK;
  if (nq >= (1 << 30)) return fail(ctx, RRTX_E_INVALID, "radius search: at most 2^30 - 1 queries per call");

  double tlt = 0.0, tgt = 0.0;
  if (!r_dev_thr_lt) {
    if (ctx->thr_cache_r != r_scalar || std::isnan(r_scalar)) {
      ctx->thr_cache_r = r_scalar;
      ctx->thr_cache_lt = thr_first_ge(r_scalar);
      ctx->thr_cache_gt = thr_first_gt(r_scalar);
    }
    tlt = ctx->thr_cache_lt;
    tgt = ctx->thr_cache_gt;
  }
  const unsigned prev_overflow = ctx->mailbox.p ? *ctx->mailbox.as<volatile unsigned>() : 0u;
  if (prev_overflow > 0 && ctx->bkt_mult < 16) ctx->bkt_mult *= 2;

  const RadiusPlan p = plan_radius(ctx, nq, cap, prev_overflow, ext != nullptr);
  int rc = radius_workspaces(ctx, p);
  if (rc) return rc;
  const int flip = ctx->scalars_flip ^ 1;
  RadiusArgs d;
  radius_args(ctx, p, flip, ext, d);
  if (p.fuse) ext->fused = true;
  ctx->last_culled = p.use_cull;
  ctx->last_placement = p.slot_route ? 2 : (p.use_cull ? 1 : 0);
  ctx->last_tile_form = p.use_cull ? (p.straight ? 2 : 1) : 0;
  ctx->last_tile_q = p.use_cull ? kTileB : p.tile_q;
  if (p.use_cull) ctx->last_visit_slices = p.n_slices;
  ctx->last_pairs = (int64_t)p.n_copies_max * p.n_nodes;

  span_begin(ctx, KF_NN_FINISH);
  for_dim(ctx->dim, [&](auto dc) {
    launch_nn_pack<decltype(dc)::value>(ctx, q_dev, nq, r_dev_thr_lt, r_dev_thr_lt ? r_dev_thr_lt + nq : nullptr, tlt,
                                        tgt, d.sc, ctx->d_xrange.as<unsigned long long>(), p.g2, p.g3, d.qhist, d.cbk,
                                        d.pf, d.ca, d.qs, d.ps);
  });
  span_end(ctx);
  ctx->scalars_flip = flip;

  if (p.use_filter && !p.slot_route) {
    span_begin(ctx, KF_NN_FINISH);
    radius_place_or_prep(ctx, p, d);
    span_end(ctx);
  }

  span_begin(ctx, KF_NN_SCAN);
  if (p.use_cull) radius_scan_tiles(ctx, p, d);
  else radius_scan_brute(ctx, p, d);
  span_end(ctx);

  span_begin(ctx, KF_NN_FINISH);
  if (p.prescatter) radius_prescatter(ctx, p, d, offsets_dev, needed_dev, cap);
  {
    FinishLaunch f;
    f.count = d.count; f.nq = nq; f.bcap = p.bcap;
    f.bkt = d.ca.hs.bkt; f.tmp = ctx->ws_tmp.p; f.ovf = ctx->ws_recs.p; f.ovf_cap = p.rec_cap; f.scalars = d.sc;
    f.prescattered = p.prescatter;
    f.offsets = offsets_dev; f.needed = needed_dev; f.idx = idx_dev; f.dist = dist_dev; f.out_cap = (long long)cap;
    f.owner = owner_dev; f.nearest_idx = nearest_idx_dev; f.nearest_dist = nearest_dist_dev;
    f.qhist = d.qhist; f.n_qhist = p.use_cull ? p.n_buckets + 1 : 0;
    f.mailbox = ctx->mailbox.as<unsigned>();
    f.q = q_dev;
    f.r_start = (!r_dev_thr_lt && r_scalar > 0.0) ? 2.0 * r_scalar : 1.0;
    f.hit_out = p.fuse ? ext->hit_out : nullptr; f.hit_in = p.fuse ? ext->hit_in : nullptr;
    rc = launch_nn_finish(ctx, f);
    if (rc) return rc;
  }
  span_end(ctx);
  RRTX_HIP(ctx, hipGetLastError());
  return RRTX_OK;
}

#ifdef RRTX_TILE_CLOCKS
extern "C" int rrtx_debug_tile_clocks(unsigned long long *out, int n_words) {
  return (int)hipMemcpyFromSymbol(out, HIP_SYMBOL(g_tile_clk), sizeof(unsigned long long) * (size_t)n_words);
}
#endif

int scan_units(rrtx_ctx *ctx, int *units) {
  std::vector<int> v((size_t)ctx->last_visit_slices);
  if (!v.empty()) {
    RRTX_HIP(ctx, hipMemcpyAsync(v.data(), ctx->ws_ev_cnt.p, sizeof(int) * v.size(), hipMemcpyDeviceToHost, ctx->stream));
    RRTX_HIP(ctx, hipStreamSynchronize(ctx->stream));
  }
  long long tot = 0;
  for (int x : v) tot += x;
  tot = (tot + kChunkF / 8 - 1) / (kChunkF / 8);
  *units = (int)(tot > 0x7fffffffll ? 0x7fffffffll : tot);
  return RRTX_OK;
}

}
```

rrtqx_3d_amd/csrc/nn_device.hpp:

```cpp
#pragma once
#include "collide_device.hpp"
#include "exact_math.hpp"
#include "rrtx_internal.hpp"
#include "wave_device.hpp"

namespace rrtx {
namespace {


constexpr int kScanU = 4;
constexpr int kScanThreads = 256;
constexpr int kChunk = 64 * kScanU;

struct Scalars {
  unsigned long long total;
  int n_copies;
  int n_units;
  unsigned long long q_absmax;
  int n_spill;
  int pad;
};

struct alignas(16) BktRec { int32_t idx; int32_t pad; double d2; };

struct HitSink {
  int *count;
  BktRec *bkt;
  int bcap;
  int pad;
  HitRec *recs;
  long long cap;
  Scalars *sc;
};

struct ConfirmArgs {
  const double *nx, *ny, *nz, *nw;
  const void *copies;
  const int2 *meta;
  const SlotRec *slots;
  const int32_t *pos_id;
  int n_slots;
  int pad;
  HitSink hs;
};

struct alignas(16) QRecF3 { float x, y, z, thr; };
struct alignas(32) QRecF4 { float x, y, z, w, thr, pad0, pad1, pad2; };
template <int D> struct QRecFT;
template <> struct QRecFT<3> { using type = QRecF3; };
template <> struct QRecFT<4> { using type = QRecF4; };

constexpr int kTileQExact = 32;
constexpr int kTileQFilter = 64;
constexpr int kScanFU = 8;
constexpr int kQPI = 4;
constexpr int kChunkF = 64 * kScanFU;

__global__ void nn_init_kernel(Scalars *__restrict__ sc, int n_copies_init, int *__restrict__ zero_i32, int n_i32,
                               unsigned long long *__restrict__ fill_u64, int n_u64, unsigned long long v_u64,
                               int *__restrict__ fill_i32, int n_fill_i32, int v_i32,
                               ConfirmArgs *__restrict__ ca_dst, ConfirmArgs ca) {
  const int i = blockIdx.x * blockDim.x + threadIdx.x;
  const int stride = gridDim.x * blockDim.x;
  if (i == 0) {
    sc->total = 0ull; sc->n_copies = n_copies_init; sc->n_units = 0; sc->q_absmax = 0ull; sc->n_spill = 0;
    if (ca_dst) *ca_dst = ca;
  }
  for (int k = i; k < n_i32; k += stride) zero_i32[k] = 0;
  for (int k = i; k < n_u64; k += stride) fill_u64[k] = v_u64;
  for (int k = i; k < n_fill_i32; k += stride) fill_i32[k] = v_i32;
}

template <int D>
__device__ __forceinline__ typename QRecFT<D>::type make_qrecf(const typename QRecT<D>::type &c, double C, double ox,
                                                               double oy, double oz, double ow) {
  const float qx = (float)(c.x - ox), qy = (float)(c.y - oy), qz = (float)(c.z - oz);
  float qw = 0.f;
  double qq = (double)qx * (double)qx + (double)qy * (double)qy + (double)qz * (double)qz;
  if constexpr (D == 4) { qw = (float)(c.w - ow); qq += (double)qw * (double)qw; }
  float thr_f;
  if (!(C <= 1e15)) {
    thr_f = __builtin_inff();
  } else if (!(c.thr > 0.0)) {
    thr_f = -__builtin_inff();
  } else {
    const double eps = 5.9604644775390625e-08;
    const double K = (D == 4) ? 42.0 : 26.0;
    const double two_sqrt_d = (D == 4) ? 4.0 : 3.4641016151377544;
    const double R = sqrt_rn(c.thr) * (1.0 + 1e-15);
    const double b = R + two_sqrt_d * eps * C * (1.0 + 1e-6);
    const double T = b * b * (1.0 + 1e-12) + K * eps * C * C + 1e-30 - qq * (1.0 - 1e-14);
    thr_f = __double2float_ru(T);
    if (thr_f != thr_f) thr_f = __builtin_inff();
  }
  typename QRecFT<D>::type f;
  f.x = -2.0f * qx; f.y = -2.0f * qy; f.z = -2.0f * qz;
  if constexpr (D == 4) { f.w = -2.0f * qw; f.pad0 = 0.f; f.pad1 = 0.f; f.pad2 = 0.f; }
  f.thr = thr_f;
  return f;
}

template <int D>
__device__ __forceinline__ typename QRecFT<D>::type never_pass_qrecf() {
  typename QRecFT<D>::type f;
  f.x = 0.f; f.y = 0.f; f.z = 0.f;
  if constexpr (D == 4) { f.w = 0.f; f.pad0 = 0.f; f.pad1 = 0.f; f.pad2 = 0.f; }
  f.thr = -__builtin_inff();
  return f;
}

template <int D>
struct alignas(64) QSlotRec {
  typename QRecT<D>::type q;
  typename QRecFT<D>::type f;
  int owner;
};
struct QSlots {
  void *tab;
  int2 *spill_key;
  const unsigned long long *node_absmax;
  int capb, spill_base;
};

struct PackFused {
  int *count;
  Scalars *sc_next;
  ConfirmArgs *ca_dst;
  const double *nx, *ny, *nz, *nw;
  const SphRec *sph;
  int m_sph;
  int root_rule;
};

struct QGrid { double x0, ix, y0, iy, z0, iz; int sx, sy, sz; };
__device__ __forceinline__ QGrid query_grid(const unsigned long long *__restrict__ xrange, int g2, int g3) {
  QGrid g;
  const double xw = dec_ord(xrange[1]) - dec_ord(xrange[0]), yw = dec_ord(xrange[3]) - dec_ord(xrange[2]);
  const double zw = dec_ord(xrange[5]) - dec_ord(xrange[4]);
  const bool use_z = g3 > 1 && zw > 0.125 * fmax(xw, yw) && zw < 1e300;
  g.sx = use_z ? g3 : g2; g.sy = g.sx; g.sz = use_z ? g3 : 1;
  slab_map(xrange[0], xrange[1], g.sx, &g.x0, &g.ix);
  slab_map(xrange[2], xrange[3], g.sy, &g.y0, &g.iy);
  slab_map(xrange[4], xrange[5], g.sz, &g.z0, &g.iz);
  return g;
}
__device__ __forceinline__ int query_bucket(const QGrid &g, double x, double y, double z) {
  const int cx = slab_of(x, g.x0, g.ix, g.sx), cy = slab_of(y, g.y0, g.iy, g.sy), cz = slab_of(z, g.z0, g.iz, g.sz);
  const int row = cz * g.sy + ((cz & 1) ? (g.sy - 1 - cy) : cy);
  return row * g.sx + ((row & 1) ? (g.sx - 1 - cx) : cx);
}

struct PackSamples {
  ExtendDev x;
  SampleList *out;
};
constexpr int kPackSampleGroups = 2;

__device__ __forceinline__ void pack_sample_role(const double *__restrict__ q, int nq, int wg, const PackSamples &ps) {
  __shared__ SampleGroupLds grp[kPackSampleGroups];
  const ExtendDev &x = ps.x;
  const int t = threadIdx.x, lane = t & 63;
  const int gi = __builtin_amdgcn_readfirstlane(t >> 7), gl = t & 127;
  SampleGroupLds &g = grp[gi];
  const int s0 = (wg * kPackSampleGroups + gi) * kSampleGroup;
  const int nsamp = max(0, min(kSampleGroup, nq - s0));
  ReachProbe rp;
  rp.mx = 0.f; rp.my = 0.f; rp.mz = 0.f; rp.h = 0.f;
  if (lane < nsamp) {
    const size_t i = (size_t)(s0 + lane);
    const double cx = q[i * 3 + 0], cy = q[i * 3 + 1], cz = q[i * 3 + 2];
    const double rb = x.r_bound >= 0.0 ? x.r_bound : 0.0;
    const double pmax = fmax(fmax(fabs(cx), fabs(cy)), fabs(cz));
    const double base_b = rb + 1e-12 * (pmax + 1.0);
    const bool usable = (pmax < 1e29) && (cx == cx) && (cy == cy) && (cz == cz) && (base_b < 1e29);
    rp = reach_probe(x, cx, cy, cz, base_b, usable);
    if (gl < kSampleGroup) {
      g.px[lane] = cx; g.py[lane] = cy; g.pz[lane] = cz; g.base[lane] = base_b;
      g.snl[lane] = 0; g.sbad[lane] = 0;
    }
  }
  __syncthreads();
  sample_pass_group(x, g, nsamp, gl, rp);
  __syncthreads();
  if (gl < nsamp) {
    const int n = g.snl[gl], bad = g.sbad[gl] ? 1 : 0;
    int l[kSphListCap];
#pragma unroll
    for (int c = 0; c < kSphListCap; ++c) l[c] = c < n ? g.ssl[gl][c] : 0;
    int4 *dst = reinterpret_cast<int4 *>(ps.out + (s0 + gl));
    dst[0] = make_int4(n, bad, 0, 0);
    dst[1] = make_int4(l[0], l[1], l[2], l[3]);
    dst[2] = make_int4(l[4], l[5], l[6], l[7]);
    if (x.sample_unsafe) x.sample_unsafe[s0 + gl] = (uint8_t)bad;
  }
}

template <int D>
__global__ void nn_pack_kernel(const double *__restrict__ q, int nq, const double *__restrict__ thr_lt_arr,
                               const double *__restrict__ thr_gt_arr, double thr_lt_s, double thr_gt_s,
                               int n_wraps, int wd0, int wd1, int wd2, double wp0, double wp1, double wp2,
                               double ox, double oy, double oz, double ow,
                               SlotRec *__restrict__ slots, typename QRecT<D>::type *__restrict__ copies,
                               int2 *__restrict__ meta, Scalars *__restrict__ sc,
                               const unsigned long long *__restrict__ xrange, int g2, int g3,
                               int *__restrict__ qhist, int2 *__restrict__ cb, PackFused pf, ConfirmArgs ca,
                               QSlots qs, PackSamples ps) {
  if constexpr (D == 3) {
    const int n_qwg = (nq + 255) / 256;
    if ((int)blockIdx.x >= n_qwg) {
      pack_sample_role(q, nq, (int)blockIdx.x - n_qwg, ps);
      return;
    }
  }
  const int i = blockIdx.x * blockDim.x + threadIdx.x;
  const bool act = i < nq;
  if (i == 0 && pf.count) {
    pf.count[nq] = 0;
    *pf.ca_dst = ca;
    Scalars *nx_sc = pf.sc_next;
    nx_sc->total = 0ull; nx_sc->n_copies = 0; nx_sc->n_units = 0; nx_sc->q_absmax = 0ull; nx_sc->n_spill = 0;
    if (n_wraps == 0) sc->n_copies = nq;
  }
  unsigned long long am = 0ull;
  if (act) {
    QGrid qg;
    if (qhist) qg = query_grid(xrange, g2, g3);
    double p[4] = {0.0, 0.0, 0.0, 0.0};
#pragma unroll
    for (int k = 0; k < D; ++k) p[k] = q[(size_t)i * D + k];
    const double tlt = thr_lt_arr ? thr_lt_arr[i] : thr_lt_s;
    const double tgt = thr_gt_arr ? thr_gt_arr[i] : thr_gt_s;
    const int n_slots = 1 << n_wraps;
    const int wd[3] = {wd0, wd1, wd2};
    const double wp[3] = {wp0, wp1, wp2};
    if (pf.count) {
      const double s = (D == 4) ? sq4(p[0], p[1], p[2], p[3], pf.nx[0], pf.ny[0], pf.nz[0], pf.nw[0])
                                : sq3(p[0], p[1], p[2], pf.nx[0], pf.ny[0], pf.nz[0]);
      const bool add = pf.root_rule && s >= tlt && s < tgt;
      pf.count[i] = add ? 1 : 0;
      if (add) {
        BktRec br;
        br.idx = 0; br.pad = 0; br.d2 = s;
        if (pf.m_sph > 0) {
          const double rx = pf.nx[0], ry = pf.ny[0], rz = pf.nz[0], len = sqrt_rn(s);
          bool ho = false, hi = false;
          for (int j = 0; j < pf.m_sph; ++j) {
            const SphRec ob = pf.sph[j];
            ho = ho || edge_hits_sphere(p[0], p[1], p[2], rx - p[0], ry - p[1], rz - p[2], len, ob);
            hi = hi || edge_hits_sphere(rx, ry, rz, p[0] - rx, p[1] - ry, p[2] - rz, len, ob);
          }
          br.pad = (ho ? 1 : 0) | (hi ? 2 : 0);
        }
        ca.hs.bkt[(size_t)i * (size_t)ca.hs.bcap] = br;
      }
    }
    for (int k = 0; k < n_slots; ++k) {
      double g[4] = {p[0], p[1], p[2], p[3]};
      double c[4] = {p[0], p[1], p[2], p[3]};
      for (int w = 0; w < n_wraps; ++w) {
        int bit = (k >> (n_wraps - 1 - w)) & 1;
        if (!bit) continue;
        int dimi = wd[w];
        double dim_val = p[dimi];
        double dim_closest = 0.0;
        if (p[dimi] < wp[w] / 2.0) { dim_val += wp[w]; dim_closest += wp[w]; }
        else { dim_val -= wp[w]; }
        g[dimi] = dim_val;
        c[dimi] = dim_closest;
      }
      bool valid = true;
      if (k > 0) {
        double s = (D == 4) ? sq4(c[0], c[1], c[2], c[3], g[0], g[1], g[2], g[3])
                            : sq3(c[0], c[1], c[2], g[0], g[1], g[2]);
        valid = !(s >= tgt);
      }
      SlotRec sr;
      sr.x = g[0]; sr.y = g[1]; sr.z = g[2]; sr.w = g[3];
      sr.thr_lt = valid ? tlt : -1.0;
      sr.thr_gt = (pf.count && !pf.root_rule) ? tlt : tgt;
      sr.pad0 = 0.0; sr.pad1 = 0.0;
      if (n_wraps > 0) slots[(size_t)i * n_slots + k] = sr;
      if (valid) {
        const double og[4] = {ox, oy, oz, ow};
        unsigned long long amc = 0ull;
        for (int c2 = 0; c2 < D; ++c2) amc = max(amc, (unsigned long long)__double_as_longlong(fabs(g[c2] - og[c2])));
        typename QRecT<D>::type qr;
        qr.x = g[0]; qr.y = g[1]; qr.z = g[2];
        if constexpr (D == 4) { qr.w = g[3]; qr.pad0 = 0.0; qr.pad1 = 0.0; qr.pad2 = 0.0; }
        qr.thr = tlt;
        if (qs.tab) {
          QSlotRec<D> rec;
          rec.q = qr;
          rec.f = make_qrecf<D>(qr, __longlong_as_double((long long)max(*qs.node_absmax, amc)), ox, oy, oz, ow);
          rec.owner = i;
          const int b = query_bucket(qg, g[0], g[1], g[2]);
          const int r = atomicAdd(&qhist[b], 1);
          QSlotRec<D> *tab = static_cast<QSlotRec<D> *>(qs.tab);
          const bool sp = r >= qs.capb;
          if (!sp) tab[(size_t)b * qs.capb + r] = rec;
          const unsigned long long m = __ballot(sp);
          if (m != 0ull) {
            const int lane = threadIdx.x & 63;
            const int leader = __ffsll((long long)m) - 1;
            int base = 0;
            if (lane == leader) base = atomicAdd(&sc->n_spill, __popcll(m));
            base = __shfl(base, leader);
            if (sp) {
              const int j = base + __popcll(m & ((1ull << lane) - 1ull));
              tab[(size_t)qs.spill_base + j] = rec;
              qs.spill_key[j] = make_int2(b, r);
            }
          }
          continue;
        }
        am = max(am, amc);
        int pos = (n_wraps == 0) ? i : atomicAdd(&sc->n_copies, 1);
        copies[pos] = qr;
        meta[pos] = make_int2(i, k);
        if (qhist) {
          const int b = query_bucket(qg, g[0], g[1], g[2]);
          cb[pos] = make_int2(b, atomicAdd(&qhist[b], 1));
        }
      }
    }
  }
#pragma unroll
  for (int off = 32; off > 0; off >>= 1) {
    const unsigned long long o = __shfl_xor(am, off);
    am = max(am, o);
  }
  if ((threadIdx.x & 63) == 0 && am != 0ull) atomicMax(&sc->q_absmax, am);
}

template <int D>
inline void launch_nn_pack(rrtx_ctx *ctx, const double *q, int nq, const double *thr_lt_arr, const double *thr_gt_arr,
                           double thr_lt_s, double thr_gt_s, Scalars *sc, const unsigned long long *xrange, int g2,
                           int g3, int *qhist, int2 *cb, const PackFused &pf, const ConfirmArgs &ca, const QSlots &qs,
                           const PackSamples &ps) {
  constexpr int kPerWg = kPackSampleGroups * kSampleGroup;
  const int n_swg = (D == 3 && ps.out) ? (nq + kPerWg - 1) / kPerWg : 0;
  hipLaunchKernelGGL(nn_pack_kernel<D>, dim3((nq + 255) / 256 + n_swg), dim3(256), 0, ctx->stream, q, nq, thr_lt_arr,
                     thr_gt_arr, thr_lt_s, thr_gt_s, ctx->n_wraps, ctx->wrap_dim[0], ctx->wrap_dim[1], ctx->wrap_dim[2],
                     ctx->wrap_period[0], ctx->wrap_period[1], ctx->wrap_period[2], ctx->origin[0], ctx->origin[1],
                     ctx->origin[2], ctx->origin[3], ctx->ws_slots.as<SlotRec>(),
                     ctx->ws_copies.as<typename QRecT<D>::type>(), ctx->ws_copy_meta.as<int2>(), sc, xrange, g2, g3,
                     qhist, cb, pf, ca, qs, ps);
}

template <int D>
__device__ __noinline__ bool seen_by_earlier_slot(const SlotRec *__restrict__ slots, int n_slots, int owner,
                                                  int slot, int node_idx, double x, double y, double z,
                                                  double w) {
  for (int j = 0; j < slot; ++j) {
    SlotRec sr = slots[(size_t)owner * n_slots + j];
    if (sr.thr_lt < 0.0) continue;
    double s = (D == 4) ? sq4(sr.x, sr.y, sr.z, sr.w, x, y, z, w) : sq3(sr.x, sr.y, sr.z, x, y, z);
    double thr = (j == 0 && node_idx == 0) ? sr.thr_gt : sr.thr_lt;
    if (s < thr) return true;
  }
  return false;
}

__device__ __forceinline__ void place_hit(const HitSink &hs, bool hit, int owner, int slot, int id, double d2,
                                          int flags = 0) {
  const bool inb = hit && slot < hs.bcap;
  if (inb) {
    const size_t at = (size_t)owner * (size_t)hs.bcap + (size_t)slot;
    BktRec br;
    br.idx = id; br.pad = flags; br.d2 = d2;
    hs.bkt[at] = br;
  }
  const bool ov = hit && !inb;
  const unsigned long long m = __ballot(ov);
  if (m != 0ull) {
    const int lane = threadIdx.x & 63;
    const int leader = __ffsll((long long)m) - 1;
    unsigned long long base = 0;
    if (lane == leader) base = atomicAdd(&hs.sc->total, (unsigned long long)__popcll(m));
    base = __shfl(base, leader);
    if (ov) {
      const long long pos = (long long)base + __popcll(m & ((1ull << lane) - 1ull));
      if (pos < hs.cap) {
        HitRec r;
        r.owner = owner | (flags << 30);
        r.idx = id; r.d2 = d2;
        hs.recs[pos] = r;
      }
    }
  }
}

__device__ __forceinline__ void emit_hit(const HitSink &hs, bool hit, int owner, int id, double d2) {
  int slot = 0;
  if (hit) slot = atomicAdd(&hs.count[owner], 1);
  place_hit(hs, hit, owner, slot, id, d2);
}

__device__ __forceinline__ void emit_hits_grouped(const HitSink &hs, bool hit, int owner, int id, double d2,
                                                  int flags = 0) {
  const int lane = threadIdx.x & 63;
  unsigned long long rem = __ballot(hit);
  while (rem != 0ull) {
    const int L = __ffsll((long long)rem) - 1;
    const int o = __builtin_amdgcn_readlane(owner, L);
    const bool mine = hit && owner == o;
    const unsigned long long m = __ballot(mine);
    int base = 0;
    if (lane == L) base = atomicAdd(&hs.count[o], __popcll(m));
    base = __builtin_amdgcn_readlane(base, L);
    place_hit(hs, mine, o, base + __popcll(m & ((1ull << lane) - 1ull)), id, d2, flags);
    rem &= ~m;
  }
}

struct GlobalEmit {
  static constexpr bool kNeedsOwner = true;
  static constexpr bool kBatch = false;
  __device__ __forceinline__ void batch(int, int, unsigned, const int *, const double *) const {}
  const HitSink &hs;
  __device__ __forceinline__ void operator()(bool h, int , int owner, int id, double d2) const {
    emit_hit(hs, h, owner, id, d2);
  }
};

template <int D>
__global__ void nn_filter_prep_kernel(const typename QRecT<D>::type *__restrict__ copies,
                                      const Scalars *__restrict__ sc,
                                      const unsigned long long *__restrict__ node_absmax, int ,
                                      double ox, double oy, double oz, double ow,
                                      typename QRecFT<D>::type *__restrict__ copies_f) {
  int i = blockIdx.x * blockDim.x + threadIdx.x;
  const int n_copies = sc->n_copies;
  if (i >= n_copies) {
    if (i < ((n_copies + kQPI - 1) / kQPI) * kQPI) copies_f[i] = never_pass_qrecf<D>();
    return;
  }
  unsigned long long cb = max(*node_absmax, sc->q_absmax);
  copies_f[i] = make_qrecf<D>(copies[i], __longlong_as_double((long long)cb), ox, oy, oz, ow);
}

constexpr int kCandCap = 192;
constexpr int kNearestWarm = 256;
typedef float f32x2 __attribute__((ext_vector_type(2)));

template <int D>
__device__ __forceinline__ void screen8(const typename QRecFT<D>::type &c, const float *x, const float *y,
                                        const float *z, const float *w, const float *pp, float *t) {
  const f32x2 cx2 = {c.x, c.x}, cy2 = {c.y, c.y}, cz2 = {c.z, c.z};
#pragma unroll
  for (int v = 0; v < kScanFU / 2; ++v) {
    f32x2 a = {pp[2 * v], pp[2 * v + 1]};
    const f32x2 xz = {z[2 * v], z[2 * v + 1]}, xy = {y[2 * v], y[2 * v + 1]}, xx = {x[2 * v], x[2 * v + 1]};
    a = __builtin_elementwise_fma(cz2, xz, a);
    if constexpr (D == 4) {
      const f32x2 cw2 = {c.w, c.w}, xw = {w[2 * v], w[2 * v + 1]};
      a = __builtin_elementwise_fma(cw2, xw, a);
    }
    a = __builtin_elementwise_fma(cy2, xy, a);
    a = __builtin_elementwise_fma(cx2, xx, a);
    t[2 * v] = a.x; t[2 * v + 1] = a.y;
  }
}

constexpr int kSlabKz = 32;

struct NearestIndex {
  const double *sx, *sy, *sz, *sw;
  const int32_t *sid;
  const ChunkExt *chunk_ext;
  int n_chunks, n_nodes;
};
struct NearestScratch { double s[16]; int i[16]; int skipped; };

template <int D, int NT>
__device__ __forceinline__ void block_nearest(const NearestIndex &ni, const double px, const double py, const double pz,
                                           const double pw, double r_start, NearestScratch &sm, double &best_s_out,
                                           int &best_i_out) {
  const int t = threadIdx.x, lane = t & 63;
  const int wave = __builtin_amdgcn_readfirstlane(t >> 6);
  constexpr int NW = NT / 64;
  const bool finite_p = (px - px == 0.0) && (py - py == 0.0) && (pz - pz == 0.0) && (D == 3 || (pw - pw == 0.0));
  double R = (r_start > 0.0 && r_start < 1e300) ? r_start : 1.0;
  if (!finite_p) R = __builtin_inf();
  double best = __builtin_inf();
  int best_i = 0x7fffffff;
  for (int it = 0;; ++it) {
    if (it >= 48) R = __builtin_inf();
    double lo = -__builtin_inf(), hi = __builtin_inf(), ylo = lo, yhi = hi;
    const bool cull = finite_p && R < 1e300;
    if (cull) {
      const double a = px - R, b = px + R, ya = py - R, yb = py + R;
      lo = a - (fabs(a) * 4.5e-16 + 1e-300);
      hi = b + (fabs(b) * 4.5e-16 + 1e-300);
      ylo = ya - (fabs(ya) * 4.5e-16 + 1e-300);
      yhi = yb + (fabs(yb) * 4.5e-16 + 1e-300);
    }
    if (t == 0) sm.skipped = 0;
    __syncthreads();
    best = __builtin_inf();
    best_i = 0x7fffffff;
    bool skipped = false;
    for (int c = wave; c < ni.n_chunks; c += NW) {
      if (cull) {
        const ChunkExt ce = ni.chunk_ext[c];
        if (!(dec_ord(ce.xhi) >= lo && dec_ord(ce.xlo) <= hi && dec_ord(ce.yhi) >= ylo && dec_ord(ce.ylo) <= yhi)) {
          skipped = true;
          continue;
        }
      }
#pragma unroll 2
      for (int u = 0; u < kChunkF / 64; ++u) {
        const int pos = c * kChunkF + u * 64 + lane;
        if (pos < ni.n_nodes) {
          double s;
          if constexpr (D == 4) s = sq4(px, py, pz, pw, ni.sx[pos], ni.sy[pos], ni.sz[pos], ni.sw[pos]);
          else s = sq3(px, py, pz, ni.sx[pos], ni.sy[pos], ni.sz[pos]);
          const int id = ni.sid[pos];
          const bool better = (s < best) || (s == best && id < best_i);
          best = better ? s : best;
          best_i = better ? id : best_i;
        }
      }
    }
#pragma unroll
    for (int off = 32; off > 0; off >>= 1) {
      const double ob = __shfl_xor(best, off);
      const int oi = __shfl_xor(best_i, off);
      if ((ob < best) || (ob == best && oi < best_i)) { best = ob; best_i = oi; }
    }
    if (lane == 0) {
      sm.s[wave] = best; sm.i[wave] = best_i;
      if (skipped) sm.skipped = 1;
    }
    __syncthreads();
    best = sm.s[0]; best_i = sm.i[0];
    for (int w = 1; w < NW; ++w) {
      const double ob = sm.s[w];
      const int oi = sm.i[w];
      if ((ob < best) || (ob == best && oi < best_i)) { best = ob; best_i = oi; }
    }
    const bool any_skipped = sm.skipped != 0;
    __syncthreads();
    if (!cull || !any_skipped) break;
    if (best < R * R * (1.0 - 1e-12)) break;
    R = R * 2.0;
  }
  best_s_out = best;
  best_i_out = best_i;
}

inline int round_up(int a, int b) { return (a + b - 1) / b * b; }

inline int pow2_ceil(long long v) {
  int p = 1;
  while (p < v && p < (1 << 30)) p <<= 1;
  return p;
}

}
}
```

rrtqx_3d_amd/csrc/rrtx_internal.hpp:

```cpp
#pragma once

#include <hip/hip_runtime.h>

#include <algorithm>
#include <cmath>
#include <cstdint>
#include <cstdio>
#include <cstring>
#include <string>
#include <type_traits>
#include <utility>
#include <vector>

#include "../../include/rrtx.h"

namespace rrtx {

constexpr int kMaxWraps = 3;
constexpr int kMaxSlots = 1 << kMaxWraps;

struct alignas(32) QRec3 { double x, y, z, thr; };
struct alignas(64) QRec4 { double x, y, z, w, thr, pad0, pad1, pad2; };
template <int D> struct QRecT;
template <> struct QRecT<3> { using type = QRec3; };
template <> struct QRecT<4> { using type = QRec4; };

struct alignas(64) SlotRec { double x, y, z, w, thr_lt, thr_gt, pad0, pad1; };

struct alignas(16) HitRec { int32_t owner; int32_t idx; double d2; };

struct alignas(32) SphRec { double cx, cy, cz, thr; };

struct alignas(64) SweepObs { SphRec ob; double thr_lt, thr_gt; int32_t active, pad0; double pad1; };

struct SweepQuery { double x, y, z, w, thr_lt, thr_root; };

struct alignas(64) SweepQueryOwned { SweepQuery q; unsigned long long owner; double pad; };

struct ChunkExtHost { unsigned long long xlo, xhi, ylo, yhi; };

template <hipError_t (*Free)(void *)>
struct Owned {
  void *p = nullptr;
  size_t bytes = 0;
  Owned() = default;
  Owned(const Owned &) = delete;
  Owned(Owned &&o) noexcept : p(o.p), bytes(o.bytes) { o.p = nullptr; o.bytes = 0; }
  Owned &operator=(Owned &&o) noexcept {
    if (this != &o) { release(); std::swap(p, o.p); std::swap(bytes, o.bytes); }
    return *this;
  }
  ~Owned() { release(); }
  void release() { if (p) (void)Free(p); p = nullptr; bytes = 0; }
  template <class T> T *as() const { return reinterpret_cast<T *>(p); }
};
struct DevBuf : Owned<hipFree> {
  size_t grown(size_t need) const {
    size_t nb = bytes ? bytes : 4096;
    while (nb < need) nb *= 2;
    return nb;
  }
  hipError_t ensure(size_t need) {
    if (need <= bytes) return hipSuccess;
    const size_t nb = grown(need);
    if (p) { hipError_t e = hipFree(p); if (e != hipSuccess) return e; p = nullptr; bytes = 0; }
    hipError_t e = hipMalloc(&p, nb);
    if (e == hipSuccess) bytes = nb;
    return e;
  }
  hipError_t regrow(size_t new_bytes, size_t keep, hipStream_t st) {
    DevBuf nb;
    hipError_t e = hipMalloc(&nb.p, new_bytes);
    if (e != hipSuccess) return e;
    nb.bytes = new_bytes;
    if (p && keep > 0) e = hipMemcpyAsync(nb.p, p, keep, hipMemcpyDeviceToDevice, st);
    if (p && e == hipSuccess) e = hipStreamSynchronize(st);
    if (e == hipSuccess) *this = std::move(nb);
    return e;
  }
  hipError_t ensure_keep(size_t need, size_t keep, hipStream_t st) {
    return need <= bytes ? hipSuccess : regrow(grown(need), keep, st);
  }
};
template <class T>
struct DevArray {
  DevBuf buf;
  T *get() const { return buf.as<T>(); }
  operator T *() const { return get(); }
  hipError_t regrow(size_t count, size_t keep, hipStream_t st) { return buf.regrow(sizeof(T) * count, sizeof(T) * keep, st); }
};
struct PinnedBuf : Owned<hipHostFree> {
  hipError_t alloc(size_t nb, unsigned flags) {
    release();
    const hipError_t e = hipHostMalloc(&p, nb, flags);
    if (e == hipSuccess) bytes = nb;
    return e;
  }
};
static_assert(!std::is_copy_constructible<DevBuf>::value && !std::is_copy_constructible<DevArray<double>>::value &&
              !std::is_copy_constructible<PinnedBuf>::value, "an allocation has one owner");

constexpr int32_t kNoParentEdge = 0x7fffffff;
constexpr int32_t kRemovedEdge = -2;

struct GraphCost {
  DevBuf lmc, parent, stamp, flags, orph, anc, ids;
  DevBuf in_cnt, in_start, in_cursor, in_tiles;
  DevBuf in_src, in_w, in_pos;
  int64_t in_ne = 0;
  int in_nn = 0;
  int solved_root = -1;
  int64_t solved_nodes = 0, solved_edges = 0;
  bool touched_old = false;
  DevBuf rep_lmc, rep_parent;
  int rep_root = -1;
  int64_t rep_nodes = 0;
  DevBuf delta_cnt, delta_pos;
};

struct SphView {
  const SphRec *rec = nullptr, *reach = nullptr;
  const float *reach_f = nullptr;
  const double *sample = nullptr;
  const double *radius = nullptr, *thr_in = nullptr;
  const int32_t *orig = nullptr;
  int m = 0;
};
struct PolyView {
  const double *meta = nullptr;
  const int32_t *off = nullptr;
  const double *vxy = nullptr, *vslope = nullptr;
  const int32_t *orig = nullptr;
  const double *bbox = nullptr, *pbox = nullptr, *ytab = nullptr;
  int n_ytab = 0;
  const int32_t *path_off = nullptr;
  const double *path = nullptr;
  int m = 0;
  bool has_moving = false;
};

enum KernelFamily { KF_NN_SCAN = 0, KF_NN_FINISH, KF_NN_NEAREST, KF_EDGES, KF_POINTS, KF_DUBINS, KF_DUBINS_STEER, KF_COUNT };

struct TimedSpan { hipEvent_t a, b; int family; };

}

struct rrtx_ctx {
  int dim = 3;
  int device = 0;
  hipStream_t own_stream = nullptr;
  rrtx::PinnedBuf h_arena;
  size_t h_arena_used = 0;
  struct HostCopy { void *dst; const void *src; size_t bytes; };
  std::vector<HostCopy> h_pending;
  std::vector<std::pair<const char *, size_t>> h_registered;
  hipStream_t stream = nullptr;
  std::string err;

  rrtx::DevArray<double> nodes[4];
  rrtx::DevArray<double> nodes_aos;
  rrtx::DevArray<float> nodes_f[4];
  rrtx::DevArray<float> nodes_pp;
  double origin[4] = {0, 0, 0, 0};
  bool origin_set = false;
  int64_t n_nodes = 0, cap_nodes = 0;
  rrtx::DevBuf d_absmax;

  rrtx::DevArray<float> sl_f[4];
  rrtx::DevArray<double> sl_d[4];
  rrtx::DevArray<float> sl_pp;
  rrtx::DevArray<int32_t> sl_id;
  rrtx::DevArray<rrtx::ChunkExtHost> chunk_ext;
  int64_t cap_chunks = 0;
  int64_t sl_n_sorted = 0;
  double sl_run_chunks = 0.0;
  int sl_cells = 0;
  int sl_kz = 0;
  double sl_debt_us = 0.0;
  rrtx::DevBuf d_xrange;
  rrtx::DevBuf ws_slab_hist, ws_slab_start, ws_slab_sr, ws_slab_params, ws_run_hist, ws_run_sr;
  int run_hist_flip = 0;

  int opt_nn_filter = 1;
  int opt_scan_blocks = 1280;
  int opt_scan_items = 2048;
  int opt_tile_q = 0;
  int opt_nn_cull = 1;
  long long opt_nearest_rec_cap = 0;
  int opt_space_has_time = 0;
  int opt_dubins_time_column = 0;
  double dubins_vmin = 0.0, dubins_vmax = 1e300;
  int opt_root_rule = 1;
  int opt_tune = 0;
  int opt_profile_every = 1;
  long long span_tick = 0;

  int n_wraps = 0;
  int wrap_dim[rrtx::kMaxWraps] = {0, 0, 0};
  double wrap_period[rrtx::kMaxWraps] = {0, 0, 0};

  std::vector<double> sph;
  std::vector<uint8_t> sph_active;
  bool sph_dirty = true;
  double sph_packed_rr = -1.0;
  rrtx::DevBuf d_sph_tab;
  rrtx::SphView sph_view;
  double sph_packed_origin[3] = {0, 0, 0};
  std::vector<int32_t> poly_off;
  std::vector<double> poly_vxy;
  std::vector<double> poly_cr;
  std::vector<uint8_t> poly_kind, poly_active;
  bool poly_dirty = true;
  rrtx::DevBuf d_poly_tab;
  rrtx::PolyView poly_view;
  rrtx::DevBuf d_poly_grid;
  std::vector<double> poly_h_meta, poly_h_bbox;
  double poly_grid_pad = -1.0;
  double poly_grid_x0 = 0.0, poly_grid_y0 = 0.0, poly_grid_inv_wx = 0.0, poly_grid_inv_wy = 0.0;
  int poly_grid_g = 0;
  rrtx::DevBuf ws_knn_off, ws_knn_idx, ws_knn_dist, ws_knn_misc;
  int opt_knn_lists = 1;
  int opt_extend_polygons = 0;
  std::vector<int32_t> poly_path_off;
  std::vector<double> poly_path;

  rrtx::DevBuf ws_q;
  rrtx::DevBuf ws_q2;
  rrtx::DevBuf ws_slots;
  rrtx::DevBuf ws_copies;
  rrtx::DevBuf ws_copies_f;
  rrtx::DevBuf ws_copy_meta;
  rrtx::DevBuf ws_copies_s, ws_meta_s;
  rrtx::DevBuf ws_cb, ws_qhist;
  rrtx::DevBuf ws_qslot;
  rrtx::DevBuf ws_bkt;
  int bkt_mult = 2;
  rrtx::PinnedBuf mailbox;
  rrtx::DevBuf ws_ev_a, ws_ev_cnt, ws_confirm_args;
  rrtx::DevBuf ws_recs;
  rrtx::DevBuf ws_counts;
  rrtx::DevBuf ws_bsum;
  rrtx::DevBuf ws_scalars;
  rrtx::DevBuf ws_scalars_nn;
  int scalars_flip = 0;
  rrtx::DevBuf ws_tmp;
  rrtx::DevBuf ws_owner;
  rrtx::DevBuf ws_dub_rec;
  rrtx::DevBuf ws_dub_ckpt;
  rrtx::DevBuf ws_out_off, ws_out_idx, ws_out_dist, ws_out_u8a, ws_out_u8b, ws_out_i32, ws_out_f64;
  rrtx::DevBuf ws_partial;
  rrtx::DevBuf ws_thr;
  rrtx::DevBuf ws_mask;
  rrtx::DevBuf ws_i32a, ws_i32b;
  rrtx::DevBuf ws_sph_lists;
  rrtx::DevBuf ws_poly_lists;
  rrtx::DevBuf ws_self;

  rrtx::DevArray<int32_t> ge_start, ge_end;
  rrtx::DevArray<double> ge_dist;
  rrtx::DevArray<double> ge_dist0;
  rrtx::DevArray<uint8_t> ge_dirty;
  rrtx::GraphCost gc;
  int64_t ge_n = 0, ge_cap = 0;
  rrtx::DevBuf ws_sweep_mark, ws_sweep_flag, ws_sweep_cnt, ws_sweep_start;
  rrtx::DevBuf ws_swb_tab, ws_swb_word, ws_swb_seg_id, ws_swb_seg_word, ws_swb_blk_n, ws_swb_cnt, ws_swb_pos, ws_swb_base, ws_swb_off;
  std::vector<rrtx::SweepObs> swb_tab_host;
  rrtx::DevBuf ws_rel_stay;
  std::vector<uint8_t> rel_stay_host;
  rrtx::DevBuf ws_pswb_q, ws_pswb_pos, ws_pswb_cand_id, ws_pswb_cand_word, ws_pswb_hit;
  std::vector<rrtx::SweepQueryOwned> pswb_q_host;
  std::vector<int32_t> pswb_pos_host;
  std::vector<int> pswb_qoff_host;
  rrtx::DevBuf ws_prel_stay;
  std::vector<int32_t> prel_stay_host;

  rrtx::DevArray<double> node_lmc;
  int64_t node_lmc_cap = 0, node_lmc_n = 0;
  rrtx::DevBuf ws_sel_cnt;
  rrtx::DevBuf ws_sel_blk;
  rrtx::DevBuf ws_sel_rwn, ws_sel_rwv, ws_sel_lmc;
  int64_t sel_list_cap = 0;
  int sel_hold_nq = -1;
  int64_t sel_hold_count = 0;
  int sel_hold_cols = 1;

  rrtx::DevBuf ws_link_cnt, ws_link_row, ws_link_res, ws_link_node, ws_link_get;
  rrtx::DevBuf ws_delta_node;

  rrtx::DevBuf ws_tgt_blk[2], ws_tgt_res;

  double thr_cache_r = -1.0, thr_cache_lt = 0.0, thr_cache_gt = 0.0;

  int profiling = 0;
  bool span_open = false;
  std::vector<rrtx::TimedSpan> spans;
  std::vector<hipEvent_t> event_pool;
  double fam_ms[rrtx::KF_COUNT] = {0};
  int64_t fam_launches[rrtx::KF_COUNT] = {0};
  int64_t last_pairs = 0, last_neighbors = 0;
  int last_tile_q = 0;
  bool last_culled = false;
  int last_placement = 0;
  int last_tile_form = 0;
  int64_t last_sweep_candidates = 0;
  int last_visit_slices = 0;

  rrtx::DevArray<uint8_t> ge_culled;
  rrtx::DevBuf ws_cull_map, ws_cull_nodes, ws_cull_cnt, ws_cull_pos, ws_cull_remap, ws_cull_res;

  ~rrtx_ctx();
};

namespace rrtx {

int fail(rrtx_ctx *ctx, int code, const char *fmt, ...);

struct ApiRange {
  explicit ApiRange(const char *name);
  ~ApiRange();
  bool active;
};

#define RRTX_HIP(ctx, expr)                                                               \
  do {                                                                                    \
    hipError_t _e = (expr);                                                               \
    if (_e != hipSuccess)                                                                 \
      return ::rrtx::fail((ctx), RRTX_E_DEVICE, "%s failed: %s (%s:%d)", #expr,           \
                          hipGetErrorString(_e), __FILE__, __LINE__);                     \
  } while (0)

struct TuneBits {
  bool xy_order;
  bool whole_chunks;
  bool place_pass;
  bool loop_form;
  int kz_bins;
  int g3_side;
  int cell_shift;
};
inline TuneBits tune_bits(const rrtx_ctx *ctx) {
  const int t = ctx->opt_tune;
  return TuneBits{(t & 1) != 0, (t & 2) != 0, (t & 4) != 0, (t & 8) != 0, (t >> 8) & 0xff, (t >> 16) & 0x1f, (t >> 24) & 3};
}

template <class Fn>
inline void for_dim(int dim, Fn &&fn) {
  if (dim == 4) fn(std::integral_constant<int, 4>{});
  else fn(std::integral_constant<int, 3>{});
}

void span_begin(rrtx_ctx *ctx, int family);
void span_end(rrtx_ctx *ctx);

double thr_first_ge(double r);
double thr_first_gt(double r);
double thr_point_clear(double robot_radius, double radius);

template <bool W>
struct EdgeColsT {
  template <class T> using P = std::conditional_t<W, T, const T> *;
  P<double> cost_out, cost_in; P<uint8_t> word_out, word_in, hit_out, hit_in;
};
template <bool W>
struct ListsT {
  template <class T> using P = std::conditional_t<W, T, const T> *;
  P<int64_t> offsets, count; P<int32_t> idx, owner; P<double> key; EdgeColsT<W> e; int64_t cap;
};
using EdgeCols = EdgeColsT<true>;
using Lists = ListsT<true>;
using ListsRO = ListsT<false>;
inline ListsRO read_only(const Lists &L) {
  return ListsRO{L.offsets, L.count, L.idx, L.owner, L.key,
                 {L.e.cost_out, L.e.cost_in, L.e.word_out, L.e.word_in, L.e.hit_out, L.e.hit_in}, L.cap};
}
struct NearTable { const double *p = nullptr; int64_t rows = 0; };
struct TreeColumn { const int32_t *tree_idx; EdgeCols e; };

struct ExtendFuse { double r; uint8_t *hit_out, *hit_in, *sample_unsafe; bool fused; };
struct FinishLaunch {
  const int *count; int nq; int bcap;
  const void *bkt; void *tmp; const void *ovf; long long ovf_cap; const void *scalars;
  bool prescattered;
  int64_t *offsets; int64_t *needed; int32_t *idx; double *dist; long long out_cap;
  int32_t *owner; int32_t *nearest_idx; double *nearest_dist;
  int *qhist; int n_qhist; unsigned *mailbox;
  const double *q; double r_start;
  uint8_t *hit_out, *hit_in;
};
int launch_nn_finish(rrtx_ctx *ctx, const FinishLaunch &f);
int launch_nn_radius(rrtx_ctx *ctx, const double *q_dev, const double *r_dev_or_null, double r_scalar,
                     int nq, int64_t *offsets_dev, int32_t *idx_dev, double *dist_dev, int64_t cap,
                     int64_t *needed_dev, int32_t *owner_dev = nullptr, int32_t *nearest_idx_dev = nullptr,
                     double *nearest_dist_dev = nullptr, ExtendFuse *ext = nullptr);
int knearest_row(int k, int64_t n_nodes);
int launch_nn_knearest(rrtx_ctx *ctx, const double *q_dev, int nq, int k, int32_t *idx_dev, double *dist_dev,
                       int32_t *count_dev);
int launch_nn_nearest(rrtx_ctx *ctx, const double *q_dev, int nq, int32_t *idx_dev, double *dist_dev,
                      bool exact = false);
int scan_units(rrtx_ctx *ctx, int *units);
int slab_refresh(rrtx_ctx *ctx, long long n_tiles);
bool slab_run_wanted(const rrtx_ctx *ctx, int64_t n);
struct SlabParams { double x0, inv_wx, y0, inv_wy, z0, inv_wz; int Kx, Ky, Kz, pad; };
struct RunRank { const SlabParams *sp; int *hist; int2 *sr; };
int slab_run_prepare(rrtx_ctx *ctx, int64_t n, RunRank *rr);
int slab_append_run(rrtx_ctx *ctx, int64_t base, int64_t n);
constexpr int kSlabChunk = 512;
int launch_edges_spheres(rrtx_ctx *ctx, const double *p0_dev, const double *p1_dev, int64_t ne,
                         double robot_radius, int obstacle_or_minus1, int obs_begin, int obs_end,
                         uint8_t *hit_dev, int32_t *first_hit_dev, const int32_t *sidx_dev = nullptr,
                         const int32_t *eidx_dev = nullptr, const uint8_t *mask_host = nullptr);
int launch_edges_polygons(rrtx_ctx *ctx, const double *p0_dev, const double *p1_dev, int64_t ne,
                          double robot_radius, int obstacle_or_minus1, int obs_begin, int obs_end,
                          uint8_t *hit_dev, int32_t *first_hit_dev);
int launch_points_spheres(rrtx_ctx *ctx, const double *p_dev, int64_t np, double robot_radius, int quick,
                          uint8_t *unsafe_dev, double *clearance_dev);
int launch_points_polygons(rrtx_ctx *ctx, const double *p_dev, int64_t np, double robot_radius,
                           uint8_t *unsafe_dev, double *clearance_dev, double list_r = -1.0,
                           const unsigned short **lists_out = nullptr, const unsigned short **list_cnt_out = nullptr);
int launch_simple_steer(rrtx_ctx *ctx, const double *s_dev, const double *g_dev, int64_t ne,
                        double *dist_dev, double *wdist_dev);
int launch_dubins_steer(rrtx_ctx *ctx, const double *s_dev, const double *g_dev, int64_t ne, double r_min,
                        double *cost_dev, uint8_t *word_dev, double *wdist_dev = nullptr,
                        double *velocity_dev = nullptr, uint8_t *valid_dev = nullptr);
int launch_dubins_edges_check(rrtx_ctx *ctx, const double *s_dev, const double *g_dev, int64_t ne,
                              double r_min, double robot_radius, double *cost_dev, uint8_t *word_dev,
                              uint8_t *hit_dev, int32_t *traj_len_dev, int pb = -1, int pe = -1);
int launch_dubins_edges_idx(rrtx_ctx *ctx, const int32_t *ids_dev, int64_t n, double r_min, double robot_radius, int pb,
                            int pe, uint8_t *hit_dev);
int launch_sweep_mark_multi(rrtx_ctx *ctx, const SweepQuery *queries_host, int nqs);
int launch_sweep_select(rrtx_ctx *ctx, int blocked_only, int32_t *out_dev, long long cap, long long **total_dev);
int launch_sweep_finish(rrtx_ctx *ctx, const int32_t *ids_dev, long long n, const uint8_t *hit, const uint8_t *o1,
                        const uint8_t *o2, int32_t *out_dev, long long cap, long long **total_dev);
int launch_sweep_gather(rrtx_ctx *ctx, const int32_t *ids_dev, long long n, double *p0_dev, double *p1_dev);
void packed_range(const std::vector<int32_t> &orig, int begin, int end, int &pb, int &pe);
std::vector<int32_t> active_positions(const std::vector<uint8_t> &active);
int launch_candidate_dubins(rrtx_ctx *ctx, const Lists &L, const double *q_dev, int nq, double r_min, double robot_radius,
                            NearTable near = {});
int launch_detmath_eval(rrtx_ctx *ctx, int op, const double *x_dev, const double *y_dev, int64_t n, double *out_dev);
int launch_dubins_trajectory(rrtx_ctx *ctx, const double *s_dev, const double *g_dev, int64_t ne, double r_min,
                             const int64_t *traj_off_dev, double *traj_xy_dev, int64_t cap_rows,
                             int32_t *traj_len_dev);
int launch_candidate_edges(rrtx_ctx *ctx, const double *q_dev, int nq, const int64_t *offsets_dev,
                           const int32_t *idx_dev, const int32_t *owner_dev, int64_t cap, double robot_radius,
                           uint8_t *hit_out_dev, uint8_t *hit_in_dev, double r = -1.0,
                           uint8_t *sample_unsafe_dev = nullptr, const double *near_aos = nullptr, int64_t n_near = 0);
int launch_candidate_edges_polygons(rrtx_ctx *ctx, const double *q_dev, int nq, const int64_t *offsets_dev,
                                    const int32_t *idx_dev, const int32_t *owner_dev, int64_t cap,
                                    double robot_radius, uint8_t *hit_out_dev, uint8_t *hit_in_dev,
                                    uint8_t *sample_unsafe_dev, double r = -1.0, const double *near_aos = nullptr,
                                    int64_t n_near = 0);
int launch_list_edges(rrtx_ctx *ctx, const Lists &L, const double *q_dev, int nq, double robot_radius, double r_min, double r,
                      NearTable near = {});
int launch_self_join(rrtx_ctx *ctx, const Lists &L, const double *q_dev, int nq, double r, const uint8_t *skip_dev,
                     NearTable *table_out);
int launch_self_join_dubins(rrtx_ctx *ctx, const Lists &L, const double *q_dev, int nq, double r, const uint8_t *skip_dev,
                            NearTable *table_out);
int launch_closest_self(rrtx_ctx *ctx, const Lists &L, const double *q_dev, int nq, int k, double robot_radius,
                        const uint8_t *skip_dev, const uint8_t *want_dev, int32_t *count_dev, const TreeColumn &tree);
int launch_closest_self_dubins(rrtx_ctx *ctx, const Lists &L, const double *q_dev, int nq, int k, double robot_radius,
                               double r_min, const uint8_t *skip_dev, const uint8_t *want_dev, int32_t *count_dev,
                               const TreeColumn &tree);
int launch_nearest_from_lists(rrtx_ctx *ctx, const ListsRO &L, int nq, int32_t *nearest_idx_dev, double *nearest_dist_dev);

int launch_obstacle_sweep(rrtx_ctx *ctx, const double centre[3], double thr_lt, double thr_gt, const SphRec &ob,
                          int active, int32_t *out_dev, int64_t cap, long long **total_dev);

int launch_sphere_burst(rrtx_ctx *ctx, int k, bool release, int32_t *out_dev, int64_t cap, long long **total_dev);

int launch_polygon_burst(rrtx_ctx *ctx, int k, double r_min, double robot_radius, bool release, int32_t *out_dev, int64_t cap,
                         long long **total_dev);
int launch_dubins_check_words(rrtx_ctx *ctx, const int32_t *cand_id, const unsigned long long *cand_word, int64_t n,
                              double r_min, double robot_radius, const int32_t *ppos_dev, int kg,
                              unsigned long long *hit_word, const int32_t *stay_dev = nullptr, int n_stay = 0);
int dubins_check_space(rrtx_ctx *ctx);

int launch_graph_edge_dist(rrtx_ctx *ctx, long long first, long long n);
int launch_graph_touch(rrtx_ctx *ctx, long long first, long long n);
int launch_graph_block(rrtx_ctx *ctx, bool restore, const int32_t *ids_host, long long n);
int launch_graph_block_dev(rrtx_ctx *ctx, bool restore, const int32_t *ids_dev, long long n);
int launch_edges_cull(rrtx_ctx *ctx, double ball, const int32_t *nodes_host, long long k, int64_t *n_culled);
int launch_edges_compact(rrtx_ctx *ctx, int32_t *remap_host, int64_t *n_removed);
int launch_graph_cost(rrtx_ctx *ctx, int root, bool update, double *lmc_dev, int32_t *parent_dev, int *passes_out);
void graph_cost_forget(rrtx_ctx *ctx);
int launch_graph_delta(rrtx_ctx *ctx, int root, bool store, int32_t *node_dev, double *lmc_dev, int32_t *par_dev, long long cap,
                       int64_t **total_dev, int *passes_out);
int launch_graph_delta_advance(rrtx_ctx *ctx, int root);
void graph_delta_forget(rrtx_ctx *ctx);

int launch_pack_hits(rrtx_ctx *ctx, const uint8_t *hit_out, const uint8_t *hit_in, const int64_t *n_valid_dev,
                     int64_t cap, uint64_t *words);

struct SelectLaunch {
  int nq;
  ListsRO lists;
  const uint8_t *sample_unsafe; const double *lmc; int64_t n_lmc;
  int32_t *parent_idx; int64_t *parent_entry; double *lmc_new; uint8_t *status;
  int64_t *rw_offsets; int32_t *rw_node; double *rw_value; int64_t rw_cap; int64_t *rw_needed_dev;
};
int launch_select(rrtx_ctx *ctx, const SelectLaunch &L);

enum : unsigned {
  kLinkOverflow = 1,
  kLinkBadNode = 2,
  kLinkBadIndex = 4,
  kLinkBadOffsets = 8,
  kLinkTooMany = 16,
};
struct LinkLists {
  int nq;
  ListsRO lists;
  const int32_t *node_of; bool idx_is_batch;
  int64_t *row_first;
};
int launch_link_count(rrtx_ctx *ctx, const LinkLists &L);
int launch_link_fill(rrtx_ctx *ctx, const LinkLists &L, long long first, long long total);
int launch_link_gather(rrtx_ctx *ctx, const int32_t *ids_dev, long long n, int32_t *start_dev, int32_t *end_dev,
                       double *dist_dev, double *dist0_dev);

struct TargetRound {
  int n_act, nq, round, dim;
  double r_max;
  const int64_t *offsets;
  const int32_t *idx; const double *cost; const uint8_t *hit_out;
  const int64_t *n_valid; long long cap;
  const double *lmc; long long n_lmc;
  const double *q, *rad; const int32_t *slot;
  int32_t *pending;
  double *cost_to_goal, *edge_dist, *radius_used; int32_t *target_idx, *rounds; uint8_t *status;
  double *q_next, *rad_next, *thr_next; int32_t *slot_next;
  int64_t *hdr;
};
int launch_target_round(rrtx_ctx *ctx, const TargetRound &T);
int node_cost_ensure(rrtx_ctx *ctx);
template <class T>
int regrow(rrtx_ctx *ctx, DevArray<T> &a, int64_t count, int64_t keep) {
  const hipError_t e = a.regrow((size_t)count, (size_t)keep, ctx->stream);
  if (e == hipErrorOutOfMemory) return fail(ctx, RRTX_E_NOMEM, "hipMalloc of %lld array elements failed", (long long)count);
  RRTX_HIP(ctx, e);
  return RRTX_OK;
}

int sync_spheres(rrtx_ctx *ctx, double robot_radius);
int sync_polygons(rrtx_ctx *ctx);
int sync_polygon_grid(rrtx_ctx *ctx, double pad_needed);

}
```

Measured before the change: 20.35 billion edges/s.

## Move fused edge collision checks from tile scan kernel into finish kernel

Moves the obstacle-sphere edge collision flag computation out of the NN tile scan kernel (where it ran per hit as hits were emitted) and into the finish kernel, which evaluates it per final neighbor after bucketing. The tile kernel loses its EXT template path, LDS sphere lists and flag packing, which should lighten the hot scan loop and its register and LDS footprint. The finish kernel gains per-query sphere lists in LDS and a second pass over large (todo) queries that re-reads idx/dist from global memory. The trade-off is extra work and an added synchronisation in the finish stage, plus removal of the root-prefill flag path.

Measured after the change: 19.09 billion edges/s. 0.938x the previous value.

```diff
diff --git a/rrtqx_3d_amd/csrc/kernels_finish.hip b/rrtqx_3d_amd/csrc/kernels_finish.hip
--- a/rrtqx_3d_amd/csrc/kernels_finish.hip
+++ b/rrtqx_3d_amd/csrc/kernels_finish.hip
@@ -1,3 +1,4 @@
+#include "collide_device.hpp"
 #include "nn_device.hpp"
 
 namespace rrtx {
@@ -37,6 +38,9 @@
   double r_start;
   NearestIndex ni;
 };
+struct FinishExtArgs : FinishArgs {
+  ExtendDev x;
+};
 
 template <int KSORT>
 struct FinLds {
@@ -56,6 +60,12 @@
   int r_besti[kFinThreads / 64];
   NearestScratch ns;
 };
+struct FinExtLds {
+  double px[kFinQ], py[kFinQ], pz[kFinQ];
+  int snl[kFinQ];
+  int sok[kFinQ];
+  SphRec ssr[kFinQ][kSphListCap];
+};
 
 __device__ __forceinline__ BktRec load_rec(const FinishArgs &a, int q, long long b, long long j) {
   if (j < a.bcap) return a.bkt[(size_t)q * (size_t)a.bcap + (size_t)j];
@@ -69,9 +79,47 @@
   return r;
 }
 
-template <int D, int KSORT>
-__global__ __launch_bounds__(kFinThreads, KSORT > kBigSort ? 2 : 8) void nn_finish_kernel(FinishArgs a) {
+struct FinSample {
+  double px, py, pz;
+  int snl, sok;
+  const SphRec *recs;
+};
+__device__ __forceinline__ double fin_uniform_d(double v) {
+  const long long b = __double_as_longlong(v);
+  const int lo = __builtin_amdgcn_readfirstlane((int)(b & 0xffffffffll)), hi = __builtin_amdgcn_readfirstlane((int)(b >> 32));
+  return __longlong_as_double(((long long)hi << 32) | (long long)(unsigned)lo);
+}
+__device__ __forceinline__ FinSample fin_sample(const FinExtLds &xs, int g) {
+  FinSample s;
+  s.px = fin_uniform_d(xs.px[g]); s.py = fin_uniform_d(xs.py[g]); s.pz = fin_uniform_d(xs.pz[g]);
+  s.snl = __builtin_amdgcn_readfirstlane(xs.snl[g]); s.sok = __builtin_amdgcn_readfirstlane(xs.sok[g]);
+  s.recs = xs.ssr[g];
+  return s;
+}
+__device__ __forceinline__ bool fin_edge_needed(const ExtendDev &x, int snl, int sok, double len) {
+  const bool quick = snl == 0 && sok != 0 && len > 0.0 && len <= x.r_bound && len < 1e29;
+  return !quick && x.m > 0;
+}
+__device__ __forceinline__ int fin_edge_flags(const ExtendDev &x, const FinSample &s, bool h, int id, double len) {
+  const bool need = h && fin_edge_needed(x, s.snl, s.sok, len);
+  if (__ballot(need) == 0ull) return 0;
+  double4 nd = make_double4(0.0, 0.0, 0.0, 0.0);
+  if (need) nd = x.naos[id];
+  bool ho, hi;
+  edge_flags(x, need, s.px, s.py, s.pz, nd.x, nd.y, nd.z, len, s.snl, nullptr, ho, hi, s.recs);
+  return (ho ? 1 : 0) | (hi ? 2 : 0);
+}
+
+template <bool EXT> struct FinArgsOf { using type = FinishArgs; };
+template <> struct FinArgsOf<true> { using type = FinishExtArgs; };
+template <int D, int KSORT, bool EXT>
+__global__ __launch_bounds__(kFinThreads, KSORT > kBigSort ? 2 : 8) void nn_finish_kernel(typename FinArgsOf<EXT>::type a) {
   __shared__ FinLds<KSORT> sm;
+  FinExtLds *xsp = nullptr;
+  if constexpr (EXT) {
+    __shared__ FinExtLds xs_lds;
+    xsp = &xs_lds;
+  }
   const int t = threadIdx.x, lane = t & 63;
   const int wave = __builtin_amdgcn_readfirstlane(t >> 6);
   const int hl = t & 31, hw = t >> 5;
@@ -94,6 +142,17 @@
   e0.idx = kInt; e0.pad = 0; e0.d2 = __builtin_inf();
   e1 = e0;
   if (qv && hl < a.bcap) e0 = a.bkt[(size_t)q * (size_t)a.bcap + (size_t)hl];
+  int x_n = 0, x_j = 0;
+  double x_px = 0.0, x_py = 0.0, x_pz = 0.0;
+  if constexpr (EXT) {
+    static_assert(D == 3, "the fused extend() route is 3-D");
+    if (qv) {
+      const SampleList *rec = a.x.lists + q;
+      x_n = rec->n;
+      if (hl < kSphListCap) x_j = rec->list[hl];
+      x_px = a.q[(size_t)q * 3 + 0]; x_py = a.q[(size_t)q * 3 + 1]; x_pz = a.q[(size_t)q * 3 + 2];
+    }
+  }
   unsigned long long psum = 0;
   if (!a.prescattered) {
     const int4 *c4 = reinterpret_cast<const int4 *>(a.count);
@@ -105,10 +164,54 @@
       psum += (unsigned)v.z + (unsigned)v.w;
     }
   }
-  const bool small = kfull <= 64 && kfull <= a.bcap;
-  const int kk = (qv && small) ? kfull : 0;
+  bool small = kfull <= 64 && kfull <= a.bcap;
+  int kk = (qv && small) ? kfull : 0;
   if (!(hl < kk)) { e0.idx = kInt; e0.d2 = __builtin_inf(); }
   if (hl + 32 < kk) e1 = a.bkt[(size_t)q * (size_t)a.bcap + (size_t)(hl + 32)];
+  int fl0 = 0, fl1 = 0;
+  if constexpr (EXT) {
+    FinExtLds &xs = *xsp;
+    if (hl == 0) {
+      const double rb = a.x.r_bound >= 0.0 ? a.x.r_bound : 0.0;
+      const double pmax = fmax(fmax(fabs(x_px), fabs(x_py)), fabs(x_pz));
+      const double base_b = rb + 1e-12 * (pmax + 1.0);
+      const bool usable = (pmax < 1e29) && (x_px == x_px) && (x_py == x_py) && (x_pz == x_pz) && (base_b < 1e29);
+      xs.px[hw] = x_px; xs.py[hw] = x_py; xs.pz[hw] = x_pz;
+      xs.snl[hw] = x_n;
+      xs.sok[hw] = (usable && a.x.r_bound >= 0.0) ? 1 : 0;
+    }
+    const bool x_listed = hl < kSphListCap && hl < x_n;
+    if (x_listed) xs.ssr[hw][hl] = a.x.sph[x_j];
+    __builtin_amdgcn_wave_barrier();
+    const int x_sok = xs.sok[hw];
+    const bool need0 = hl < kk && fin_edge_needed(a.x, x_n, x_sok, sqrt_rn(e0.d2));
+    const bool need1 = hl + 32 < kk && fin_edge_needed(a.x, x_n, x_sok, sqrt_rn(e1.d2));
+    const unsigned long long nm = __ballot(need0 || need1);
+    if (nm != 0ull) {
+      sm.s_idx[t] = e0.idx; sm.s_idx[kFinThreads + t] = e1.idx;
+      sm.s_d2[t] = e0.d2; sm.s_d2[kFinThreads + t] = e1.d2;
+      sm.s_idx[2 * kFinThreads + t] = kfull;
+      sm.s_d2[2 * kFinThreads + t] = __longlong_as_double((long long)psum);
+      sm.s_fl[t] = 0; sm.s_fl[kFinThreads + t] = 0;
+      asm volatile("" ::: "memory");
+#pragma unroll 1
+      for (int h = 0; h < 2; ++h) {
+        if ((unsigned)(nm >> (32 * h)) == 0u) continue;
+        const int src = (lane >> 5) * kFinThreads + 64 * wave + 32 * h + (lane & 31);
+        const int id = sm.s_idx[src];
+        const FinSample smp = fin_sample(xs, 2 * wave + h);
+        sm.s_fl[src] = (unsigned char)fin_edge_flags(a.x, smp, id != kInt, id, sqrt_rn(sm.s_d2[src]));
+      }
+      asm volatile("" ::: "memory");
+      fl0 = sm.s_fl[t]; fl1 = sm.s_fl[kFinThreads + t];
+      e0.idx = sm.s_idx[t]; e1.idx = sm.s_idx[kFinThreads + t];
+      e0.d2 = sm.s_d2[t]; e1.d2 = sm.s_d2[kFinThreads + t];
+      kfull = sm.s_idx[2 * kFinThreads + t];
+      psum = (unsigned long long)__double_as_longlong(sm.s_d2[2 * kFinThreads + t]);
+      small = kfull <= 64 && kfull <= a.bcap;
+      kk = (qv && small) ? kfull : 0;
+    }
+  }
   __builtin_amdgcn_wave_barrier();
 
   const int m0 = e0.idx, m1 = e1.idx;
@@ -166,32 +269,41 @@
   }
 
   {
+    int qs = q, hl2 = hl + 32;
+    if constexpr (EXT) {
+      int tb = (int)threadIdx.x;
+      asm volatile("" : "+v"(tb));
+      qs = q0 + (tb >> 5);
+      hl2 = (tb & 31) + 32;
+    }
     const long long b = qv ? sm.off[hw] : 0;
-    const bool w0 = hl < kk && b + r0 < a.out_cap, w1 = hl + 32 < kk && b + r1 < a.out_cap;
+    const bool w0 = hl < kk && b + r0 < a.out_cap, w1 = hl2 < kk && b + r1 < a.out_cap;
     const bool near = a.nearest_idx != nullptr;
     if (hl < kk) {
       const double s0 = sqrt_rn(d0);
       if (w0) {
         a.idx[b + r0] = m0;
         a.dist[b + r0] = s0;
-        if (a.owner) a.owner[b + r0] = q;
-        if (a.hit_out) { a.hit_out[b + r0] = e0.pad & 1; a.hit_in[b + r0] = (e0.pad >> 1) & 1; }
-      }
-      if (near && m0 == nbest_i && d0 == nbest) { a.nearest_idx[q] = m0; a.nearest_dist[q] = s0; }
-    }
-    if (hl + 32 < kk) {
+        if (a.owner) a.owner[b + r0] = qs;
+        if constexpr (EXT) { a.hit_out[b + r0] = fl0 & 1; a.hit_in[b + r0] = (fl0 >> 1) & 1; }
+        else if (a.hit_out) { a.hit_out[b + r0] = e0.pad & 1; a.hit_in[b + r0] = (e0.pad >> 1) & 1; }
+      }
+      if (near && m0 == nbest_i && d0 == nbest) { a.nearest_idx[qs] = m0; a.nearest_dist[qs] = s0; }
+    }
+    if (hl2 < kk) {
       const double s1 = sqrt_rn(d1);
       if (w1) {
         a.idx[b + r1] = m1;
         a.dist[b + r1] = s1;
-        if (a.owner) a.owner[b + r1] = q;
-        if (a.hit_out) { a.hit_out[b + r1] = e1.pad & 1; a.hit_in[b + r1] = (e1.pad >> 1) & 1; }
-      }
-      if (near && m1 == nbest_i && d1 == nbest) { a.nearest_idx[q] = m1; a.nearest_dist[q] = s1; }
+        if (a.owner) a.owner[b + r1] = qs;
+        if constexpr (EXT) { a.hit_out[b + r1] = fl1 & 1; a.hit_in[b + r1] = (fl1 >> 1) & 1; }
+        else if (a.hit_out) { a.hit_out[b + r1] = e1.pad & 1; a.hit_in[b + r1] = (e1.pad >> 1) & 1; }
+      }
+      if (near && m1 == nbest_i && d1 == nbest) { a.nearest_idx[qs] = m1; a.nearest_dist[qs] = s1; }
     }
     if (near && qv && small && hl == 0 && kk == 0) {
       if (a.want_nearest_fix) atomicOr(&sm.empty_mask, 1u << hw);
-      else { a.nearest_idx[q] = -1; a.nearest_dist[q] = __builtin_inf(); }
+      else { a.nearest_idx[qs] = -1; a.nearest_dist[qs] = __builtin_inf(); }
     }
   }
   __syncthreads();
@@ -314,7 +426,9 @@
           a.dist[gb + rank] = sqrt_rn(d2);
           if (a.owner) a.owner[gb + rank] = qq;
           if ((d2 < best) || (d2 == best && my < best_i)) { best = d2; best_i = my; }
-          if (a.hit_out) { a.hit_out[gb + rank] = my_fl[e] & 1; a.hit_in[gb + rank] = (my_fl[e] >> 1) & 1; }
+          if constexpr (!EXT) {
+            if (a.hit_out) { a.hit_out[gb + rank] = my_fl[e] & 1; a.hit_in[gb + rank] = (my_fl[e] >> 1) & 1; }
+          }
         }
       }
      }
@@ -363,7 +477,9 @@
           a.dist[gb + i] = sqrt_rn(d2);
           if (a.owner) a.owner[gb + i] = qq;
           if ((d2 < best) || (d2 == best && my < best_i)) { best = d2; best_i = my; }
-          if (a.hit_out) { const int fl = sm.s_fl[i]; a.hit_out[gb + i] = fl & 1; a.hit_in[gb + i] = (fl >> 1) & 1; }
+          if constexpr (!EXT) {
+            if (a.hit_out) { const int fl = sm.s_fl[i]; a.hit_out[gb + i] = fl & 1; a.hit_in[gb + i] = (fl >> 1) & 1; }
+          }
         }
       }
     } else {
@@ -380,7 +496,9 @@
           a.dist[gb + rank] = sqrt_rn(d2);
           if (a.owner) a.owner[gb + rank] = qq;
           if ((d2 < best) || (d2 == best && my < best_i)) { best = d2; best_i = my; }
-          if (a.hit_out) { a.hit_out[gb + rank] = r.pad & 1; a.hit_in[gb + rank] = (r.pad >> 1) & 1; }
+          if constexpr (!EXT) {
+            if (a.hit_out) { a.hit_out[gb + rank] = r.pad & 1; a.hit_in[gb + rank] = (r.pad >> 1) & 1; }
+          }
         }
       }
     }
@@ -404,6 +522,37 @@
       }
     }
     __syncthreads();
+  }
+
+  if constexpr (EXT) {
+    if (sm.todo_mask != 0u) {
+      asm volatile("s_waitcnt vmcnt(0)" ::: "memory");
+      __syncthreads();
+    }
+    for (unsigned tm = sm.todo_mask; tm != 0u; tm &= tm - 1u) {
+      const int g = __ffs((int)tm) - 1;
+      const long long gb = __double_as_longlong(fin_uniform_d(__longlong_as_double(sm.off[g])));
+      long long ge = gb + __builtin_amdgcn_readfirstlane(sm.kfull[g]);
+      if (ge > a.out_cap) ge = a.out_cap;
+      const int gk = ge > gb ? (int)(ge - gb) : 0;
+      const FinSample smp = fin_sample(*xsp, g);
+      for (int i0 = 0; i0 < gk; i0 += kFinThreads) {
+        const int i = i0 + t;
+        const bool act = i < gk;
+        int id = 0;
+        double len = 0.0;
+        if (act) {
+          id = __hip_atomic_load(a.idx + gb + i, __ATOMIC_RELAXED, __HIP_MEMORY_SCOPE_AGENT);
+          len = __longlong_as_double((long long)__hip_atomic_load(
+              reinterpret_cast<const unsigned long long *>(a.dist + gb + i), __ATOMIC_RELAXED, __HIP_MEMORY_SCOPE_AGENT));
+        }
+        const int fl = fin_edge_flags(a.x, smp, act && (unsigned)id < (unsigned)a.ni.n_nodes, id, len);
+        int ta = (int)threadIdx.x;
+        asm volatile("" : "+v"(ta));
+        const long long at = gb + i0 + ta;
+        if (i0 + ta < gk) { a.hit_out[at] = fl & 1; a.hit_in[at] = (fl >> 1) & 1; }
+      }
+    }
   }
 
   if (a.nearest_idx && a.want_nearest_fix) {
@@ -425,7 +574,7 @@
 
 int launch_nn_finish(rrtx_ctx *ctx, const FinishLaunch &f) {
   const int D = ctx->dim;
-  FinishArgs a;
+  FinishExtArgs a{};
   a.count = f.count; a.nq = f.nq; a.bcap = f.bcap;
   a.bkt = reinterpret_cast<const BktRec *>(f.bkt);
   a.tmp = reinterpret_cast<BktRec *>(f.tmp);
@@ -449,11 +598,19 @@
   a.hit_out = f.hit_out; a.hit_in = f.hit_in;
   const dim3 grid((unsigned)((f.nq + kFinQ - 1) / kFinQ)), block(kFinThreads);
   const bool huge = f.out_cap / (f.nq > 0 ? f.nq : 1) > 512;
-  for_dim(D, [&](auto dc) {
-    constexpr int DD = decltype(dc)::value;
-    if (huge) hipLaunchKernelGGL((nn_finish_kernel<DD, kHugeSort>), grid, block, 0, ctx->stream, a);
-    else hipLaunchKernelGGL((nn_finish_kernel<DD, kBigSort>), grid, block, 0, ctx->stream, a);
-  });
+  if (f.ext_dev) {
+    if (D != 3 || !f.hit_out || !f.hit_in || !f.q) return fail(ctx, RRTX_E_STATE, "nn_finish: fused route without its arrays");
+    a.x = *static_cast<const ExtendDev *>(f.ext_dev);
+    if (huge) hipLaunchKernelGGL((nn_finish_kernel<3, kHugeSort, true>), grid, block, 0, ctx->stream, a);
+    else hipLaunchKernelGGL((nn_finish_kernel<3, kBigSort, true>), grid, block, 0, ctx->stream, a);
+  } else {
+    const FinishArgs &base = a;
+    for_dim(D, [&](auto dc) {
+      constexpr int DD = decltype(dc)::value;
+      if (huge) hipLaunchKernelGGL((nn_finish_kernel<DD, kHugeSort, false>), grid, block, 0, ctx->stream, base);
+      else hipLaunchKernelGGL((nn_finish_kernel<DD, kBigSort, false>), grid, block, 0, ctx->stream, base);
+    });
+  }
   RRTX_HIP(ctx, hipGetLastError());
   return RRTX_OK;
 }
diff --git a/rrtqx_3d_amd/csrc/kernels_nn.hip b/rrtqx_3d_amd/csrc/kernels_nn.hip
--- a/rrtqx_3d_amd/csrc/kernels_nn.hip
+++ b/rrtqx_3d_amd/csrc/kernels_nn.hip
@@ -399,10 +399,6 @@
   typename QRecFT<D>::type cf[kTileB];
   int own[kTileB];
   BktRec hrec[kTileB][kTbLcap];
-  int snl[kTileB];
-  int sok[kTileB];
-  int ssl[kTileB][kSphListCap];
-  SphRec ssr[kTileB][kSphListCap];
 };
 
 struct TileGrid {
@@ -414,31 +410,6 @@
 };
 
 template <int D>
-__device__ __forceinline__ bool tile_edge_needed(const ExtendDev &x, const TileLds<D> &sm, int cl, double d2) {
-  const double len = sqrt_rn(d2);
-  const bool quick = sm.snl[cl] == 0 && sm.sok[cl] != 0 && len > 0.0 && len <= x.r_bound && len < 1e29;
-  return !quick && x.m > 0;
-}
-template <int D>
-__device__ __forceinline__ int tile_edge_eval(const ExtendDev &x, const TileLds<D> &sm, bool need, int cl,
-                                              const double4 nd, double d2) {
-  if (__ballot(need) == 0ull) return 0;
-  const typename QRecT<D>::type c = sm.cp[cl];
-  bool ho, hi;
-  edge_flags(x, need, c.x, c.y, c.z, nd.x, nd.y, nd.z, sqrt_rn(d2), sm.snl[cl], sm.ssl[cl], ho, hi, sm.ssr[cl]);
-  return (ho ? 1 : 0) | (hi ? 2 : 0);
-}
-template <int D>
-__device__ __forceinline__ int tile_edge_flags(const ExtendDev &x, const TileLds<D> &sm, bool h, int cl, int id,
-                                               double d2) {
-  const bool need = h && tile_edge_needed<D>(x, sm, cl, d2);
-  if (__ballot(need) == 0ull) return 0;
-  double4 nd = make_double4(0.0, 0.0, 0.0, 0.0);
-  if (need) nd = x.naos[id];
-  return tile_edge_eval<D>(x, sm, need, cl, nd, d2);
-}
-
-template <int D, bool EXT>
 struct TileEmit {
   static constexpr bool kNeedsOwner = false;
   static constexpr bool kBatch = true;
@@ -464,17 +435,15 @@
       for (int u = 0; u < 4; ++u) {
         const bool sp = (spill >> u) & 1u;
         if (__ballot(sp) == 0ull) continue;
-        int owner = 0, flags = 0;
+        int owner = 0;
         if (sp) owner = meta ? meta[q].x : sm.own[cl];
-        if constexpr (EXT) flags = tile_edge_flags<D>(x, sm, sp, cl, id[u], d2[u]);
-        emit_hits_grouped(hs, sp, owner, id[u], d2[u], flags);
+        emit_hits_grouped(hs, sp, owner, id[u], d2[u]);
       }
     }
   }
   TileLds<D> &sm;
   const HitSink &hs;
   const int2 *meta;
-  const ExtendDev &x;
   int q0;
   __device__ __forceinline__ void operator()(bool h, int q, int , int id, double d2) const {
     const int cl = h ? q - q0 : 0;
@@ -488,10 +457,9 @@
     }
     const bool spill = h && !in_lds;
     if (__ballot(spill) != 0ull) {
-      int owner = 0, flags = 0;
+      int owner = 0;
       if (spill) owner = meta ? meta[q].x : sm.own[cl];
-      if constexpr (EXT) flags = tile_edge_flags<D>(x, sm, spill, cl, id, d2);
-      emit_hits_grouped(hs, spill, owner, id, d2, flags);
+      emit_hits_grouped(hs, spill, owner, id, d2);
     }
   }
 };
@@ -558,13 +526,13 @@
   }
 }
 
-template <int D, bool EXT, bool SL, bool ONE>
+template <int D, bool SL, bool ONE>
 __global__ __launch_bounds__(kScanThreads, 4) void nn_tile_kernel(
     const float *__restrict__ fx, const float *__restrict__ fy, const float *__restrict__ fz,
     const float *__restrict__ fw, const float *__restrict__ fpp, int n_nodes, int n_chunks,
     const ChunkExt *__restrict__ chunk_ext, const typename QRecT<D>::type *__restrict__ copies_s, const typename QRecFT<D>::type *__restrict__ copies_f,
     const Scalars *__restrict__ sc, int n_parts, int2 *__restrict__ ev, int slice_cap,
-    const ConfirmArgs a, const ConfirmArgs *__restrict__ ca, const TileGrid tg, const ExtendDev x,
+    const ConfirmArgs a, const ConfirmArgs *__restrict__ ca, const TileGrid tg,
     int *__restrict__ visits, const int n_copies_known, const TilePlace tp) {
   __shared__ TileLds<D> sm;
   const int t = threadIdx.x, lane = t & 63;
@@ -678,13 +646,6 @@
           c = copies_s[q0 + lane];
         }
         sm.cp[lane] = c;
-        if constexpr (EXT) {
-          const double rb = x.r_bound >= 0.0 ? x.r_bound : 0.0;
-          const double pmax = fmax(fmax(fabs(c.x), fabs(c.y)), fabs(c.z));
-          const double base_b = rb + 1e-12 * (pmax + 1.0);
-          const bool usable = (pmax < 1e29) && (c.x == c.x) && (c.y == c.y) && (c.z == c.z) && (base_b < 1e29);
-          sm.sok[lane] = (usable && x.r_bound >= 0.0) ? 1 : 0;
-        }
         const bool can_hit = (c.thr > 0.0) && (c.x - c.x == 0.0) && (c.y - c.y == 0.0) && (c.z - c.z == 0.0);
         if (can_hit) {
           const double R = sqrt_rn(c.thr) * (1.0 + 1e-15);
@@ -788,26 +749,8 @@
               listed_to = max(listed_to, __builtin_amdgcn_readlane(run, 63));
             }
           }
-        } else if (EXT && wave >= 2) {
-          if (cb == 0) {
-            static_assert(kTileB * kSphListCap == 128, "two waves: one lane per (copy, list slot)");
-            int ts = t - 128;
-            asm volatile("" : "+v"(ts));
-            const int cl = ts / kSphListCap, ls = ts % kSphListCap;
-            int n = 0, j = 0;
-            if (cl < q1 - q0) {
-              const int owner = SL ? sm.own[cl] : a.meta[q0 + cl].x;
-              if (owner >= 0) {
-                const SampleList *rec = x.lists + owner;
-                n = rec->n; j = rec->list[ls];
-              }
-            }
-            if (ls == 0) sm.snl[cl] = n;
-            if (ls < n) { sm.ssl[cl][ls] = j; sm.ssr[cl][ls] = x.sph[j]; }
-          }
         } else {
-          const int nt = EXT ? 64 : 192;
-          for (int c = max(cb, tg.n_sorted_chunks) + (t - 64); c < ce; c += nt) {
+          for (int c = max(cb, tg.n_sorted_chunks) + (t - 64); c < ce; c += 192) {
             const ChunkExt cx = chunk_ext[c];
             if (dec_ord(cx.xhi) >= lo && dec_ord(cx.xlo) <= hi && dec_ord(cx.yhi) >= ylo && dec_ord(cx.ylo) <= yhi)
               sm.list[atomicAdd(&sm.n_list, 1)] = c;
@@ -828,7 +771,7 @@
             const bool valid = gi < G;
             const unsigned p_lane = valid ? 8u * (unsigned)sm.glist[gi] : 0u;
             if (wn + 64 * kTileB > slice_cap) {
-              const TileEmit<D, EXT> emit_now{sm, a.hs, SL ? nullptr : a.meta, x, q0};
+              const TileEmit<D> emit_now{sm, a.hs, SL ? nullptr : a.meta, q0};
               drain_slice_to<D, true>(mine, wn, n_nodes, a, emit_now, sm.cp, q0);
             }
             scan_chunk_f32<D, 2, SL>(fx, fy, fz, fw, fpp, 0, n_nodes, copies_f, q0, q1, mine, wn, p_lane, __ballot(valid),
@@ -845,7 +788,7 @@
               continue;
           }
           if (wn + 64 * kTileB > slice_cap) {
-            const TileEmit<D, EXT> emit_now{sm, a.hs, SL ? nullptr : a.meta, x, q0};
+            const TileEmit<D> emit_now{sm, a.hs, SL ? nullptr : a.meta, q0};
             drain_slice_to<D, true>(mine, wn, n_nodes, a, emit_now, sm.cp, q0);
           }
           scan_chunk_f32<D, 1, SL>(fx, fy, fz, fw, fpp, chunk * kChunkF, n_nodes, copies_f, q0, q1, mine, wn, 0u, ~0ull,
@@ -865,7 +808,7 @@
     __builtin_amdgcn_fence(__ATOMIC_SEQ_CST, "workgroup");
     __syncthreads();
     RRTX_TILE_CLK(4);
-    const TileEmit<D, EXT> emit{sm, a.hs, SL ? nullptr : a.meta, x, q0};
+    const TileEmit<D> emit{sm, a.hs, SL ? nullptr : a.meta, q0};
     const int c0 = sm.wcnt[0], c1 = c0 + sm.wcnt[1], c2 = c1 + sm.wcnt[2], total = c2 + sm.wcnt[3];
     for (int e0 = 0; e0 < total; e0 += kScanThreads) {
       const int e = e0 + t;
@@ -906,9 +849,7 @@
           BktRec br;
           br.idx = 0; br.pad = 0; br.d2 = 0.0;
           if (h) br = sm.hrec[cl][j];
-          int flags = 0;
-          if constexpr (EXT) flags = tile_edge_flags<D>(x, sm, h, h ? cl : 0, br.idx, br.d2);
-          place_hit(a.hs, h, owner, base + j, br.idx, br.d2, flags);
+          place_hit(a.hs, h, owner, base + j, br.idx, br.d2);
         }
       }
     }
@@ -987,11 +928,11 @@
   for (long long i = (long long)blockIdx.x * blockDim.x + threadIdx.x; i < total;
        i += (long long)gridDim.x * blockDim.x) {
     HitRec r = recs[i];
-    const int owner = r.owner & 0x3fffffff;
+    const int owner = r.owner;
     long long dst = offsets[owner] + bcap + atomicAdd(&cursor[owner], 1);
     if (dst < out_cap) {
       BktRec br;
-      br.idx = r.idx; br.pad = (int)((unsigned)r.owner >> 30); br.d2 = r.d2;
+      br.idx = r.idx; br.pad = 0; br.d2 = r.d2;
       tmp[dst] = br;
     }
   }
@@ -1172,7 +1113,7 @@
   d.ca_dev = ctx->ws_confirm_args.as<ConfirmArgs>();
   d.pf.count = d.count; d.pf.sc_next = ctx->ws_scalars.as<Scalars>() + (flip ^ 1); d.pf.ca_dst = d.ca_dev;
   d.pf.nx = ctx->nodes[0]; d.pf.ny = ctx->nodes[1]; d.pf.nz = ctx->nodes[2]; d.pf.nw = ctx->nodes[wi];
-  d.pf.sph = nullptr; d.pf.m_sph = -1; d.pf.root_rule = ctx->opt_root_rule;
+  d.pf.root_rule = ctx->opt_root_rule;
   d.xd.r_bound = -1.0;
   if (p.fuse) {
     const SphView &S = ctx->sph_view;
@@ -1181,7 +1122,6 @@
     d.xd.ox = ctx->origin[0]; d.xd.oy = ctx->origin[1]; d.xd.oz = ctx->origin[2]; d.xd.m = S.m;
     d.xd.r_bound = (ext->r >= 0.0 && d.xd.m > 0) ? ext->r * (1.0 + 1e-12) : -1.0;
     d.xd.sample_unsafe = ext->sample_unsafe;
-    d.pf.sph = d.xd.sph; d.pf.m_sph = d.xd.m;
     d.xd.lists = ctx->ws_sph_lists.as<SampleList>();
     d.ps.x = d.xd; d.ps.out = ctx->ws_sph_lists.as<SampleList>();
   }
@@ -1217,27 +1157,20 @@
   tpl.qhist = d.qhist; tpl.tab = d.qs.tab; tpl.spill_key = d.qs.spill_key;
   tpl.n_buckets = p.n_buckets; tpl.capb = p.capb; tpl.spill_base = p.spill_base; tpl.n_tab = p.n_tab;
   const int wi = ctx->dim == 4 ? 3 : 2;
-#define RRTX_TILE_LAUNCH_F(DD, EE, SS, OO)                                                                             \
-  hipLaunchKernelGGL((nn_tile_kernel<DD, EE, SS, OO>), dim3(p.scan_grid), dim3(kScanThreads), 0, ctx->stream,          \
+#define RRTX_TILE_LAUNCH_F(DD, SS, OO)                                                                             \
+  hipLaunchKernelGGL((nn_tile_kernel<DD, SS, OO>), dim3(p.scan_grid), dim3(kScanThreads), 0, ctx->stream,          \
                      ctx->sl_f[0], ctx->sl_f[1], ctx->sl_f[2], ctx->sl_f[wi], ctx->sl_pp, p.n_nodes, p.n_chunks,       \
                      reinterpret_cast<const ChunkExt *>(ctx->chunk_ext.get()),                                               \
                      SS ? nullptr : ctx->ws_copies_s.as<typename QRecT<DD>::type>(),                                   \
                      SS ? nullptr : ctx->ws_copies_f.as<typename QRecFT<DD>::type>(), d.sc, p.n_parts,                 \
-                     ctx->ws_ev_a.as<int2>(), p.slice_cap, d.ca, d.ca_dev, tg, d.xd, ctx->ws_ev_cnt.as<int>(),         \
+                     ctx->ws_ev_a.as<int2>(), p.slice_cap, d.ca, d.ca_dev, tg, ctx->ws_ev_cnt.as<int>(),               \
                      p.n_slots == 1 ? p.nq : -1, tpl)
-#define RRTX_TILE_LAUNCH(DD, EE, SS)                                                                                   \
-  do { if (p.straight) RRTX_TILE_LAUNCH_F(DD, EE, SS, true); else RRTX_TILE_LAUNCH_F(DD, EE, SS, false); } while (0)
+#define RRTX_TILE_LAUNCH(DD, SS)                                                                                   \
+  do { if (p.straight) RRTX_TILE_LAUNCH_F(DD, SS, true); else RRTX_TILE_LAUNCH_F(DD, SS, false); } while (0)
   for_dim(ctx->dim, [&](auto dc) {
     constexpr int D = decltype(dc)::value;
-    if constexpr (D == 3) {
-      if (p.fuse) {
-        if (p.slot_route) RRTX_TILE_LAUNCH(3, true, true);
-        else RRTX_TILE_LAUNCH(3, true, false);
-        return;
-      }
-    }
-    if (p.slot_route) RRTX_TILE_LAUNCH(D, false, true);
-    else RRTX_TILE_LAUNCH(D, false, false);
+    if (p.slot_route) RRTX_TILE_LAUNCH(D, true);
+    else RRTX_TILE_LAUNCH(D, false);
   });
 #undef RRTX_TILE_LAUNCH
 #undef RRTX_TILE_LAUNCH_F
@@ -1354,6 +1287,7 @@
     f.q = q_dev;
     f.r_start = (!r_dev_thr_lt && r_scalar > 0.0) ? 2.0 * r_scalar : 1.0;
     f.hit_out = p.fuse ? ext->hit_out : nullptr; f.hit_in = p.fuse ? ext->hit_in : nullptr;
+    f.ext_dev = p.fuse ? &d.xd : nullptr;
     rc = launch_nn_finish(ctx, f);
     if (rc) return rc;
   }
diff --git a/rrtqx_3d_amd/csrc/nn_device.hpp b/rrtqx_3d_amd/csrc/nn_device.hpp
--- a/rrtqx_3d_amd/csrc/nn_device.hpp
+++ b/rrtqx_3d_amd/csrc/nn_device.hpp
@@ -127,8 +127,6 @@
   Scalars *sc_next;
   ConfirmArgs *ca_dst;
   const double *nx, *ny, *nz, *nw;
-  const SphRec *sph;
-  int m_sph;
   int root_rule;
 };
 
@@ -241,16 +239,6 @@
       if (add) {
         BktRec br;
         br.idx = 0; br.pad = 0; br.d2 = s;
-        if (pf.m_sph > 0) {
-          const double rx = pf.nx[0], ry = pf.ny[0], rz = pf.nz[0], len = sqrt_rn(s);
-          bool ho = false, hi = false;
-          for (int j = 0; j < pf.m_sph; ++j) {
-            const SphRec ob = pf.sph[j];
-            ho = ho || edge_hits_sphere(p[0], p[1], p[2], rx - p[0], ry - p[1], rz - p[2], len, ob);
-            hi = hi || edge_hits_sphere(rx, ry, rz, p[0] - rx, p[1] - ry, p[2] - rz, len, ob);
-          }
-          br.pad = (ho ? 1 : 0) | (hi ? 2 : 0);
-        }
         ca.hs.bkt[(size_t)i * (size_t)ca.hs.bcap] = br;
       }
     }
@@ -361,13 +349,12 @@
   return false;
 }
 
-__device__ __forceinline__ void place_hit(const HitSink &hs, bool hit, int owner, int slot, int id, double d2,
-                                          int flags = 0) {
+__device__ __forceinline__ void place_hit(const HitSink &hs, bool hit, int owner, int slot, int id, double d2) {
   const bool inb = hit && slot < hs.bcap;
   if (inb) {
     const size_t at = (size_t)owner * (size_t)hs.bcap + (size_t)slot;
     BktRec br;
-    br.idx = id; br.pad = flags; br.d2 = d2;
+    br.idx = id; br.pad = 0; br.d2 = d2;
     hs.bkt[at] = br;
   }
   const bool ov = hit && !inb;
@@ -382,7 +369,7 @@
       const long long pos = (long long)base + __popcll(m & ((1ull << lane) - 1ull));
       if (pos < hs.cap) {
         HitRec r;
-        r.owner = owner | (flags << 30);
+        r.owner = owner;
         r.idx = id; r.d2 = d2;
         hs.recs[pos] = r;
       }
@@ -396,8 +383,7 @@
   place_hit(hs, hit, owner, slot, id, d2);
 }
 
-__device__ __forceinline__ void emit_hits_grouped(const HitSink &hs, bool hit, int owner, int id, double d2,
-                                                  int flags = 0) {
+__device__ __forceinline__ void emit_hits_grouped(const HitSink &hs, bool hit, int owner, int id, double d2) {
   const int lane = threadIdx.x & 63;
   unsigned long long rem = __ballot(hit);
   while (rem != 0ull) {
@@ -408,7 +394,7 @@
     int base = 0;
     if (lane == L) base = atomicAdd(&hs.count[o], __popcll(m));
     base = __builtin_amdgcn_readlane(base, L);
-    place_hit(hs, mine, o, base + __popcll(m & ((1ull << lane) - 1ull)), id, d2, flags);
+    place_hit(hs, mine, o, base + __popcll(m & ((1ull << lane) - 1ull)), id, d2);
     rem &= ~m;
   }
 }
diff --git a/rrtqx_3d_amd/csrc/rrtx_internal.hpp b/rrtqx_3d_amd/csrc/rrtx_internal.hpp
--- a/rrtqx_3d_amd/csrc/rrtx_internal.hpp
+++ b/rrtqx_3d_amd/csrc/rrtx_internal.hpp
@@ -386,6 +386,7 @@
   int *qhist; int n_qhist; unsigned *mailbox;
   const double *q; double r_start;
   uint8_t *hit_out, *hit_in;
+  const void *ext_dev;
 };
 int launch_nn_finish(rrtx_ctx *ctx, const FinishLaunch &f);
 int launch_nn_radius(rrtx_ctx *ctx, const double *q_dev, const double *r_dev_or_null, double r_scalar,
```
